# reglab/aquaculture

Hardware: AMD Instinct MI355X
Metric: 640px tiles/sec (whole node) YOLOv5m bf16 (higher is better)
Workload: dtype bf16

## Files before the change

### aquaculture_amd/csrc/bottleneck.hip

```cpp
#include "conv_device.h"

using namespace aqdev;

namespace {

struct BtlParams {
    const char* in;
    char* out;
    const char* w;
    const float* bias;
    int in_ld_b, out_ld_b;
    int B, H, W;
    int tiles_x, tiles_y, n_tiles;
    int shortcut;
    unsigned long long* debug;
    const char* zero;
};

template <int MBW, int MSPLIT, int NW, int TW, int KT, bool W1REG, bool RESG> struct BtlGeom {
    static constexpr int C = 16 * MBW * MSPLIT;
    static constexpr int CB = C / 8;
    static constexpr int PG = NW / MSPLIT;
    static constexpr int TH = 4 * PG;
    static constexpr int PH = TH + 2, PW = TW + 2, PP = PH * PW;
// ... 503 lines not shown

void btl_asm_pack(const float* w1, const float* w2, bf16_t* dst) {
    const int C = 48;
    static const int pairs[5][2] = {{0, 1}, {3, 4}, {6, 7}, {2, 5}, {8, -1}};
    for (int s = 0; s < 2; ++s)
        for (int m = 0; m < 3; ++m)
            for (int lane = 0; lane < 64; ++lane, dst += 8) {
                const int co = 16 * m + (lane & 15), blk = 4 * s + (lane >> 4);
                for (int e = 0; e < 8; ++e) dst[e] = blk < 6 ? aq_f2bf(w1[(size_t)co * C + blk * 8 + e]) : aq_f2bf(0.0f);
            }
    for (int s = 0; s < 14; ++s)
        for (int m = 0; m < 3; ++m)
            for (int lane = 0; lane < 64; ++lane, dst += 8) {
                const int co = 16 * m + (lane & 15), g = lane >> 4;
                int tap, c0;
                if (s < 9) { tap = s; c0 = 8 * g; }
                else { tap = pairs[s - 9][g >> 1]; c0 = 32 + 8 * (g & 1); }
                for (int e = 0; e < 8; ++e) dst[e] = tap >= 0 ? aq_f2bf(w2[((size_t)co * 9 + tap) * C + c0 + e]) : aq_f2bf(0.0f);
            }
}

const unsigned char kBtl96AsmCode[] = {
#include "bottleneck96_asm_hsaco.inc"
};
constexpr size_t kBtl96AsmWBytes = (size_t)2 * (9 + 81) * 1024;

bool btl96_asm_fits(int C, int B, int H, int W, int in_ld, int out_ld) {
    static const bool off = [] { const char* e = getenv("AQ_BTL96_ASM"); return e && *e == '0'; }();
    if (C != 96 || off || !btl_asm_enabled() || btl_wide()) return false;
    const long long tx = (W + 15) / 16, ty = (H + 7) / 8, tpi = tx * ty, nt = tpi * B;
    if (tx < 2 || tpi < 2 || nt >= (1LL << 24) || nt * tpi >= (1LL << 32)) return false;
    if ((long long)B * H * W * in_ld * 2 >= (1LL << 30) || (long long)B * H * W * out_ld * 2 >= (1LL << 31)) return false;
    return true;
}

int launch_btl96_asm(const BtlParams& p, hipStream_t stream) {
    int cus = 0;
    AQ_CHECK_HIP(aq_cus(&cus));
    BtlAsmArgs a{};
    a.in = p.in; a.out = p.out; a.bias = p.bias;
    a.w = p.w;
    a.in_ld_b = p.in_ld_b; a.out_ld_b = p.out_ld_b; a.B = p.B; a.H = p.H; a.W = p.W;
    a.tiles_x = (p.W + 15) / 16;
    a.tpi = a.tiles_x * ((p.H + 7) / 8);
    a.ntiles = a.tpi * p.B;
    a.shortcut = p.shortcut;
    long long grid = cus;
    if (grid > a.ntiles) grid = a.ntiles;
    a.G = (int)grid;
    a.magic_tpi = (unsigned)((1ULL << 32) / (unsigned)a.tpi + 1);
    a.magic_tx = (unsigned)((1ULL << 32) / (unsigned)a.tiles_x + 1);
    a.in_bytes = (unsigned)(((long long)p.B * p.H * p.W - 1) * p.in_ld_b + 192);
    a.pad = (unsigned)(((long long)p.B * p.H * p.W - 1) * p.out_ld_b + 192);
    a.debug = aq_stamp_target((size_t)grid * 4 * 64);
    const char* exp_kernel = getenv("AQ_BTL96_ASM_KERNEL");
    char name[96];
    snprintf(name, sizeof name, "%s%s", exp_kernel && *exp_kernel ? exp_kernel : "bottleneck_asm_c96", a.debug ? "_stamped" : "");
    hipFunction_t fn = nullptr;
    AQ_CHECK_HIP(aq_asm_fn(kBtl96AsmCode, name, &fn, false));
    AQ_CHECK_HIP(aq_asm_launch(fn, (unsigned)grid, 256, &a, sizeof a, stream));
    return AQ_OK;
}

void btl96_asm_pack(const float* w1, const float* w2, bf16_t* dst) {
    const int C = 96;
    for (int h = 0; h < 2; ++h) {
        auto chan = [&](int m, int r) { return 48 * h + (m < 2 ? 8 * (r >> 2) + 4 * m + (r & 3) : 32 + 4 * (r >> 2) + (r & 3)); };
        for (int s = 0; s < 3; ++s)
            for (int m = 0; m < 3; ++m)
                for (int lane = 0; lane < 64; ++lane, dst += 8) {
                    const int co = chan(m, lane & 15), c0 = 32 * s + 8 * (lane >> 4);
                    for (int e = 0; e < 8; ++e) dst[e] = aq_f2bf(w1[(size_t)co * C + c0 + e]);
                }
        for (int tap = 0; tap < 9; ++tap)
            for (int s = 0; s < 3; ++s)
                for (int m = 0; m < 3; ++m)
                    for (int lane = 0; lane < 64; ++lane, dst += 8) {
                        const int co = chan(m, lane & 15), c0 = 32 * s + 8 * (lane >> 4);
                        for (int e = 0; e < 8; ++e) dst[e] = aq_f2bf(w2[((size_t)co * 9 + tap) * C + c0 + e]);
                    }
    }
}

}

extern "C" int aq_pack_bottleneck_weights(const float* w1_host, const float* w2_host, int C, void* packed_dev, size_t* bytes, void* stream) {
    BtlShape sh;
    AQ_REQUIRE(w1_host && w2_host && bytes && btl_shape(C, &sh), "pack_bottleneck: C must be 16, 32, 48, 64 or 96 (got %d)", C);
    const int cb = C / 8, ks1 = (cb + 3) / 4, ks2 = (9 * cb + 3) / 4;
    const size_t frags = (size_t)sh.msplit * (ks1 + ks2) * sh.mbw;
    const size_t hip_bytes = frags * 64 * 16;
    *bytes = hip_bytes + (C == 48 ? kBtlAsmWBytes : C == 96 ? kBtl96AsmWBytes : 0);
    if (!packed_dev) return AQ_OK;
    bf16_t* host = (bf16_t*)calloc(1, *bytes);
    AQ_REQUIRE(host, "pack_bottleneck: out of host memory");
    for (int mh = 0; mh < sh.msplit; ++mh)
        for (int s = 0; s < ks1 + ks2; ++s)
            for (int m = 0; m < sh.mbw; ++m)
                for (int lane = 0; lane < 64; ++lane) {
                    const int co = (mh * sh.mbw + m) * 16 + (lane & 15), g = lane >> 4;
                    bf16_t* dst = host + ((((size_t)mh * (ks1 + ks2) + s) * sh.mbw + m) * 64 + lane) * 8;
                    if (s < ks1) {
                        const int blk = 4 * s + g;
                        if (blk < cb)
                            for (int e = 0; e < 8; ++e) dst[e] = aq_f2bf(w1_host[(size_t)co * C + blk * 8 + e]);
                    } else {
                        const int blk = 4 * (s - ks1) + g;
                        if (blk < 9 * cb) {
                            const int tap = blk / cb, c8 = blk % cb;
                            for (int e = 0; e < 8; ++e) dst[e] = aq_f2bf(w2_host[((size_t)co * 9 + tap) * C + c8 * 8 + e]);
                        }
                    }
                }
    if (C == 48) btl_asm_pack(w1_host, w2_host, (bf16_t*)((char*)host + hip_bytes));
    if (C == 96) btl96_asm_pack(w1_host, w2_host, (bf16_t*)((char*)host + hip_bytes));
    hipError_t e = hipMemcpyAsync(packed_dev, host, *bytes, hipMemcpyHostToDevice, (hipStream_t)stream);
    if (e == hipSuccess) e = hipStreamSynchronize((hipStream_t)stream);
    free(host);
    AQ_CHECK_HIP(e);
    return AQ_OK;
}

extern "C" int aq_bottleneck(const void* in_dev, int in_ld, int in_choff, void* out_dev, int out_ld, int out_choff, int C,
                             const void* packed_w_dev, const float* bias_dev, int B, int H, int W, int shortcut, void* stream) {
    BtlShape sh;
    AQ_REQUIRE(in_dev && out_dev && packed_w_dev && bias_dev, "bottleneck: null pointer");
    AQ_REQUIRE(btl_shape(C, &sh), "bottleneck: C must be 16, 32, 48, 64 or 96 (got %d)", C);
    AQ_REQUIRE(B > 0 && H > 0 && W > 0, "bottleneck: empty input");
    AQ_REQUIRE(in_ld % 8 == 0 && out_ld % 8 == 0 && in_choff % 8 == 0 && out_choff % 8 == 0 && in_choff + C <= in_ld && out_choff + C <= out_ld,
               "bottleneck: channel slices must be 8-aligned and inside their rows");
    AQ_REQUIRE((long long)B * H * W < (1LL << 31), "bottleneck: batch too large");
    BtlParams p{};
    p.in = (const char*)in_dev + (size_t)in_choff * 2; p.in_ld_b = in_ld * 2;
    p.out = (char*)out_dev + (size_t)out_choff * 2; p.out_ld_b = out_ld * 2;
    {
        const char* i0 = (const char*)in_dev; const char* i1 = i0 + (size_t)B * H * W * in_ld * 2;
        const char* o0 = (const char*)out_dev; const char* o1 = o0 + (size_t)B * H * W * out_ld * 2;
        AQ_REQUIRE(o1 <= i0 || i1 <= o0, "bottleneck: output overlaps input");
    }
    p.w = (const char*)packed_w_dev; p.bias = bias_dev;
    p.B = B; p.H = H; p.W = W; p.shortcut = shortcut;
    p.zero = aq_zero_page();
    AQ_REQUIRE(p.zero, "bottleneck: zero page allocation failed");
    const hipStream_t st = (hipStream_t)stream;
    if (btl_asm_fits(C, B, H, W, in_ld, out_ld)) {
        BtlShape sh48;
        btl_shape(48, &sh48);
        p.w += (size_t)sh48.msplit * ((48 / 8 + 3) / 4 + (9 * 48 / 8 + 3) / 4) * sh48.mbw * 64 * 16;
        return launch_btl_asm(p, st);
    }
    if (btl96_asm_fits(C, B, H, W, in_ld, out_ld)) {
        const int cb = 96 / 8, ks1 = (cb + 3) / 4, ks2 = (9 * cb + 3) / 4;
        p.w += (size_t)sh.msplit * (ks1 + ks2) * sh.mbw * 64 * 16;
        return launch_btl96_asm(p, st);
    }
    switch (C) {
        case 16: return launch_btl<1, 1, 4, 32, 0, false, false>(p, st);
        case 32: return launch_btl<2, 1, 4, 16, 0, false, false>(p, st);
        case 48: return btl_wide() ? launch_btl<3, 1, 4, 16, 0, false, false>(p, st) : launch_btl<1, 3, 12, 16, 0, true, false>(p, st);
        case 64: return launch_btl<4, 1, 4, 16, 3, false, false>(p, st);
        default: return btl_wide() ? launch_btl<3, 2, 4, 16, 3, false, false>(p, st) : launch_btl<1, 6, 12, 16, 12, true, true>(p, st);
    }
}
```

### aquaculture_amd/csrc/engine.cpp

```cpp
#include "aq_common.h"
#include <unistd.h>
#include <string>

#include <cstdarg>
#include <cstdio>
#include <cstdlib>
#include <cstring>
#include <string>
#include <atomic>
#include <dlfcn.h>
#include <vector>

namespace {
thread_local char g_err[512] = "";
}

void aq_set_error(const char* fmt, ...) {
    va_list ap;
    va_start(ap, fmt);
    vsnprintf(g_err, sizeof(g_err), fmt, ap);
    va_end(ap);
}

extern "C" const char* aq_last_error(void) { return g_err; }
extern "C" int aq_version(void) { return 8; }

namespace {

inline size_t align_up(size_t v, size_t a) { return (v + a - 1) / a * a; }
constexpr size_t kAlign = 256;
constexpr int kCoutSlack = 256;

struct Roctx {
    int (*push)(const char*) = nullptr;
    int (*pop)() = nullptr;
    bool tried = false;
    bool on() {
        if (!tried) {
            tried = true;
            const char* v = getenv("AQ_ROCTX");
            if (v && *v == '1') {
                void* h = dlopen("librocprofiler-sdk-roctx.so", RTLD_NOW | RTLD_GLOBAL);
                if (!h) h = dlopen("libroctx64.so", RTLD_NOW | RTLD_GLOBAL);
                if (h) {
                    push = (int (*)(const char*))dlsym(h, "roctxRangePushA");
                    pop = (int (*)())dlsym(h, "roctxRangePop");
                }
            }
        }
        return push && pop;
    }
} g_roctx;

constexpr int kCountStride = 1024;

struct PackedW {
    void* w = nullptr;
    float* bias = nullptr;
    int kgroups = 0, kgroups_pad = 0, G = 0, cout_rows = 0;
    bool x3 = false;
    void* w_direct = nullptr;
    int direct_cfg = -1;
    void* w_head = nullptr;
    void* w_pl8 = nullptr;
    float* sb_pl8 = nullptr;
    void* w_f8 = nullptr;
    float* sb_f8 = nullptr;
    float act_scale = 0.0f;
    int f8_consumer = -1;
    std::vector<float> w_host, b_host;
};

void pack_host(const float* w, int cout, int k, int cin, int precision, std::vector<unsigned char>& out,
               int* kgroups, int* kgroups_pad, int* G, int* cout_rows) {
    const int eb = aq_elem_bytes(precision);
    const int g = cin * eb / 16;
    const int kg = k * k * g;
    const int kgp = (kg + 7) / 8 * 8;
    const int rows = (cout + kCoutSlack + 31) / 32 * 32;
    out.assign((size_t)rows * kgp * 16, 0);
    const int kelems = k * k * cin;
    for (int co = 0; co < cout; ++co) {
        unsigned char* dst = out.data() + (size_t)co * kgp * 16;
        const float* src = w + (size_t)co * kelems;
        if (precision == AQ_FP32) {
            memcpy(dst, src, (size_t)kelems * 4);
        } else {
            bf16_t* d = (bf16_t*)dst;
            for (int e = 0; e < kelems; ++e) d[e] = aq_f2bf(src[e]);
        }
    }
    *kgroups = kg; *kgroups_pad = kgp; *G = g; *cout_rows = rows;
}

uint16_t f2h(float f) {
    _Float16 h = (_Float16)f;
    uint16_t u;
    memcpy(&u, &h, 2);
    return u;
}
float h2f(uint16_t u) {
    _Float16 h;
    memcpy(&h, &u, 2);
    return (float)h;
}

void pack_host_x3(const float* w, const float* bias, int cout, int k, int cin, std::vector<unsigned char>& out, std::vector<float>& bias_scale,
                  int* kgroups, int* kgroups_pad, int* G, int* cout_rows) {
    const int g = cin * 4 / 16;
    const int kg = k * k * g;
    const int kgp = (kg + 7) / 8 * 8;
    const int rows = (cout + kCoutSlack + 31) / 32 * 32;
    out.assign((size_t)rows * kgp * 16, 0);
    bias_scale.assign((size_t)2 * rows, 0.0f);
    for (int r = 0; r < rows; ++r) bias_scale[rows + r] = 1.0f;
    const int kelems = k * k * cin;
    for (int co = 0; co < cout; ++co) {
        const float* src = w + (size_t)co * kelems;
        float amax = 0.0f;
        for (int e = 0; e < kelems; ++e) amax = fmaxf(amax, fabsf(src[e]));
        int sexp = 0;
        if (amax > 0.0f && std::isfinite(amax)) {
            int ex = 0;
            frexpf(amax, &ex);
            sexp = 15 - ex;
            sexp = sexp > 60 ? 60 : (sexp < -60 ? -60 : sexp);
        }
        const float sc = ldexpf(1.0f, sexp);
        bias_scale[co] = bias ? bias[co] * sc : 0.0f;
        bias_scale[rows + co] = ldexpf(1.0f, -sexp);
        uint16_t* dst = (uint16_t*)(out.data() + (size_t)co * kgp * 16);
        for (int e0 = 0; e0 < kelems; e0 += 8) {
            for (int e = 0; e < 8; ++e) {
                const float v = src[e0 + e] * sc;
                const uint16_t hi = f2h(v);
                dst[2 * e0 + e] = hi;
                dst[2 * e0 + 8 + e] = f2h(v - h2f(hi));
            }
        }
    }
    *kgroups = kg; *kgroups_pad = kgp; *G = g; *cout_rows = rows;
}

struct TensorPlace { size_t offset = 0; size_t bytes = 0; int h = 0, w = 0, elem = 0; };

}

struct aq_engine {
    int device = 0;
    aq_model_desc desc{};
    std::vector<aq_tensor_desc> tensors;
    std::vector<aq_op_desc> ops;
    std::vector<PackedW> packed;
// ... 155 lines not shown
    const int out_f32 = e->tensors[op.dst.tensor].dtype == AQ_T_F32;
    ConvParams p{};
    p.in = tptr(e, ws, tiles, op.src.tensor) + (size_t)op.src.ch_off * eb;
    p.in_ld_b = e->tensors[op.src.tensor].channels * eb;
    p.out = tptr(e, ws, tiles, op.dst.tensor) + (size_t)op.dst.ch_off * pd.elem;
    p.out_ld_b = e->tensors[op.dst.tensor].channels * pd.elem;
    if (op.res.tensor >= 0) {
        p.res = tptr(e, ws, tiles, op.res.tensor) + (size_t)op.res.ch_off * eb;
        p.res_ld_b = e->tensors[op.res.tensor].channels * eb;
    }
    p.w = (const char*)pw.w; p.bias = pw.bias; p.zero = (const char*)e->zero_page;
    p.B = B; p.H = ps.h; p.W = ps.w; p.Ho = pd.h; p.Wo = pd.w;
    p.cout = op.dst.channels;
    p.k = op.k; p.stride = op.stride; p.pad = op.pad; p.taps = op.k * op.k;
    p.G = pw.G; p.kgroups = pw.kgroups; p.kgroups_pad = pw.kgroups_pad; p.nchunks = pw.kgroups_pad / 8;
    p.npix = B * pd.h * pd.w;
    p.act = op.act;
    int cfg = force_cfg >= 0 ? force_cfg : e->conv_cfg[oi];
    if (cfg < 0 && tt) cfg = tt->cfg[oi];
    if (cfg == AQ_CONV_CFG_DIRECT3X3S2) {
        if (pw.direct_cfg != cfg) { aq_set_error("conv op %d has no direct 3x3/s2 form", oi); return AQ_ERR_INVALID; }
        note_launch(e, oi, AQ_FAM_DIRECT3X3S2, cfg);
        return aq_conv3x3s2_direct(tptr(e, ws, tiles, op.src.tensor), e->tensors[op.src.tensor].channels, op.src.ch_off,
                                   tptr(e, ws, tiles, op.dst.tensor), e->tensors[op.dst.tensor].channels, op.dst.ch_off,
                                   op.src.channels, op.dst.channels, pw.w_direct, pw.bias, B, ps.h, ps.w, op.act, stream);
    }
    if (cfg == AQ_CONV_CFG_PL3X3) {
        if (pw.direct_cfg != cfg) { aq_set_error("conv op %d has no planar 3x3 form", oi); return AQ_ERR_INVALID; }
        const int ld = e->tensors[op.src.tensor].channels;
        note_launch(e, oi, pw.w_pl8 && aq_conv3x3_pl_w8_supported(op.src.channels, op.dst.channels, B, ps.h, ps.w) ? AQ_FAM_PL3X3_W8 : AQ_FAM_PL3X3, cfg);
        if (pw.w_pl8 && aq_conv3x3_pl_w8_supported(op.src.channels, op.dst.channels, B, ps.h, ps.w))
            return aq_conv3x3_pl_w8(tptr(e, ws, tiles, op.src.tensor) + (size_t)op.src.ch_off * 2, (long long)ld * 2, 16, op.src.channels,
                                    tptr(e, ws, tiles, op.dst.tensor), e->tensors[op.dst.tensor].channels, op.dst.ch_off, op.dst.channels,
                                    op.res.tensor >= 0 ? tptr(e, ws, tiles, op.res.tensor) : nullptr,
                                    op.res.tensor >= 0 ? e->tensors[op.res.tensor].channels : 0, op.res.ch_off,
                                    pw.w_pl8, pw.sb_pl8, B, ps.h, ps.w, op.act, stream);
        return aq_conv3x3_pl_at(tptr(e, ws, tiles, op.src.tensor) + (size_t)op.src.ch_off * 2, (long long)ld * 2, 16, op.src.channels,
                                tptr(e, ws, tiles, op.dst.tensor), e->tensors[op.dst.tensor].channels, op.dst.ch_off, op.dst.channels,
                                op.res.tensor >= 0 ? tptr(e, ws, tiles, op.res.tensor) : nullptr,
                                op.res.tensor >= 0 ? e->tensors[op.res.tensor].channels : 0, op.res.ch_off,
                                pw.w_direct, pw.bias, B, ps.h, ps.w, op.act, tt ? tt->B : B, stream);
    }
    if (cfg == AQ_CONV_CFG_PL3X3S2) {
        if (pw.direct_cfg != cfg) { aq_set_error("conv op %d has no planar 3x3/s2 form", oi); return AQ_ERR_INVALID; }
        if (!aq_conv3x3_pl_s2_supported(op.src.channels, op.dst.channels, B, ps.h, ps.w)) {
            aq_set_error("conv op %d: planar 3x3/s2 does not fit %d x %d x %d", oi, B, ps.h, ps.w);
            return AQ_ERR_INVALID;
        }
        note_launch(e, oi, AQ_FAM_PL3X3S2, cfg);
        return aq_conv3x3_pl_s2(tptr(e, ws, tiles, op.src.tensor), e->tensors[op.src.tensor].channels, op.src.ch_off, op.src.channels,
                                tptr(e, ws, tiles, op.dst.tensor), e->tensors[op.dst.tensor].channels, op.dst.ch_off, op.dst.channels,
                                pw.w_direct, pw.bias, B, ps.h, ps.w, op.act, stream);
    }
    if (cfg == AQ_CONV_CFG_DIRECT1X1) {
        if (pw.direct_cfg != cfg) { aq_set_error("conv op %d has no direct 1x1 form", oi); return AQ_ERR_INVALID; }
        note_launch(e, oi, AQ_FAM_DIRECT1X1, cfg);
        return aq_conv1x1_direct(tptr(e, ws, tiles, op.src.tensor), e->tensors[op.src.tensor].channels, op.src.ch_off,
                                 tptr(e, ws, tiles, op.dst.tensor), e->tensors[op.dst.tensor].channels, op.dst.ch_off,
                                 op.src.channels, op.dst.channels, pw.w_direct, pw.bias, (long long)B * pd.h * pd.w, op.act, stream);
    }
    if (cfg == AQ_CONV_CFG_ASM1X1) {
        if (pw.direct_cfg != cfg) { aq_set_error("conv op %d has no assembly 1x1 form", oi); return AQ_ERR_INVALID; }
        note_launch(e, oi, AQ_FAM_ASM1X1, cfg);
        return aq_conv1x1_asm(tptr(e, ws, tiles, op.src.tensor), e->tensors[op.src.tensor].channels, op.src.ch_off,
                              tptr(e, ws, tiles, op.dst.tensor), e->tensors[op.dst.tensor].channels, op.dst.ch_off,
                              op.src.channels, op.dst.channels, pw.w_direct, pw.bias, (long long)B * pd.h * pd.w, op.act, stream);
    }
    if (cfg < 0) cfg = aq_conv_pick_config(p.cout, p.npix, prec);
    if (pw.x3) p.x3_off = pw.cout_rows;
    note_launch(e, oi, AQ_FAM_IGEMM_OR_HALO, cfg);
    return aq_launch_conv(p, pw.x3 ? (int)AQ_F16X3 : prec, out_f32, cfg, stream);
}

bool heads_fused(const aq_engine* e) {
    int n_heads = 0;
    for (size_t oi = 0; oi < e->ops.size(); ++oi)
        if (e->ops[oi].kind == AQ_OP_CONV && e->ops[oi].level >= 0) {
            ++n_heads;
            if (!e->packed[oi].w_head) return false;
        }
    return n_heads == 3;
}

struct AugRun {
    int pass;
    const aq_augment_pass* ps;
    int H0, W0;
    const aq_tap* ytab;
    const aq_tap* xtab;
};

int run_plan(aq_engine* e, const uint8_t* tiles, int B, int H, int W, void* ws, size_t ws_bytes,
             float* pred_out, aq_det* dets, int32_t* counts, float conf, float iou, int max_det, hipStream_t stream,
             int first = 0, int last = -1, const AugRun* ar = nullptr) {
    AQ_REQUIRE(e && tiles && ws, "infer: null pointer");
    const int n_ops = (int)e->ops.size();
    if (last < 0) last = n_ops;
    AQ_REQUIRE(0 <= first && first <= last && last <= n_ops, "run_ops: range [%d, %d) is not inside the plan's %d ops", first, last, n_ops);
    int rc = AQ_OK;
    if (!ar) {
        rc = layout(e, B, H, W);
        if (rc) return rc;
        if (ws_bytes < e->total_bytes) {
            aq_set_error("workspace too small: need %zu bytes, got %zu", e->total_bytes, ws_bytes);
            return AQ_ERR_WORKSPACE;
        }
    }
    const bool scaled = ar && ar->pass > 0;
    const int aug_base = ar ? ar->ps->out_first - ar->ps->keep_first : 0;
    const float aug_scale = ar ? ar->ps->scale : 1.0f, aug_flip_w = ar && ar->ps->flip ? (float)ar->W0 : 0.0f;
    e->last_ws = ws; e->last_tiles = tiles;
    const int prec = e->desc.precision;
    const bool whole = first == 0 && last == n_ops;
    hipEvent_t* ev = nullptr;
    if (whole && !ar && e->prof && e->ring > 0) ev = e->ev.data() + (size_t)(e->prof_calls % e->ring) * (n_ops + 1);
    float* pred = pred_out ? pred_out : (float*)((char*)ws + e->off_pred);
    int32_t* cand = (int32_t*)((char*)ws + e->off_cand);
    int32_t* cand_count = (int32_t*)((char*)ws + e->off_cand_count);
    float* cand_rows = (float*)((char*)ws + e->off_cand_rows);
    const char* use_sd = getenv("AQ_STEMDOWN");
    const bool stemdown = use_sd && *use_sd == '1' && prec == AQ_BF16 && n_ops > 2 && e->ops[0].kind == AQ_OP_STEM && e->ops[1].kind == AQ_OP_DOWNBLOCK &&
                          e->ops[0].dst.channels == 48 && e->ops[1].src.tensor == e->ops[0].dst.tensor && e->ops[1].src.ch_off == e->ops[0].dst.ch_off &&
                          aq_stemdown_supported(H, W) && ((uintptr_t)tiles & 3) == 0 && !scaled;
    const bool fuse_heads = dets != nullptr && heads_fused(e);
    bool heads_started = ar != nullptr;
    int heads_done = 0;
    for (int oi = 0; oi < first; ++oi)
        if (fuse_heads && e->ops[oi].kind == AQ_OP_CONV && e->ops[oi].level >= 0) {
            heads_started = true;
            ++heads_done;
        }
    for (int oi = first; oi < last; ++oi) {
        const aq_op_desc& op = e->ops[oi];
        if (ev) AQ_CHECK_HIP(hipEventRecord(ev[oi], stream));
        const bool mark = g_roctx.on();
        if (mark) {
            char name[96];
            snprintf(name, sizeof name, "aq op %02d kind %d: %d -> %d ch, k%d s%d%s", oi, op.kind, op.src.channels, op.dst.channels, op.k, op.stride,
                     op.level >= 0 ? " (detect head)" : "");
            g_roctx.push(name);
        }
        switch (op.kind) {
        case AQ_OP_PREPROCESS:
            if (scaled)
                rc = aq_preprocess_s2d_scaled(tiles, ar->H0, ar->W0, ar->ytab, ar->xtab, ar->ps->h, ar->ps->w, tptr(e, ws, tiles, op.dst.tensor), B, H, W,
                                              prec, stream);
            else
                rc = aq_preprocess_s2d(tiles, tptr(e, ws, tiles, op.dst.tensor), B, H, W, prec, stream);
            break;
        case AQ_OP_CONV:
            if (ar && op.level >= 0 && !((ar->ps->level_mask >> op.level) & 1)) {
                note_launch(e, oi, AQ_FAM_NONE);
                break;
            }
            if (fuse_heads && op.level >= 0) {
                int32_t* wide = (int32_t*)((char*)ws + e->off_cand_wide);
                if (!heads_started) {
                    AQ_CHECK_HIP(hipMemsetAsync(wide, 0, sizeof(int32_t) * B * kCountStride, stream));
                    heads_started = true;
                }
                const TensorPlace& pl = e->place[op.src.tensor];
                int off = 0;
                for (int l = 0; l < op.level; ++l) off += e->desc.na * (H / (int)e->desc.stride[l]) * (W / (int)e->desc.stride[l]);
                float anchors[8 * 2];
                for (int a = 0; a < e->desc.na; ++a) {
                    anchors[2 * a] = e->desc.anchors_px[op.level][a][0];
                    anchors[2 * a + 1] = e->desc.anchors_px[op.level][a][1];
                }
                note_launch(e, oi, AQ_FAM_HEAD_DECODE);
                if (ar) {
                    rc = aq_head_decode_aug(tptr(e, ws, tiles, op.src.tensor), e->tensors[op.src.tensor].channels, op.src.ch_off, op.src.channels,
                                            e->packed[oi].w_head, B, pl.h, pl.w, aug_base + off, e->desc.stride[op.level], anchors, e->desc.nc, e->desc.na,
                                            conf, aug_scale, aug_flip_w, cand, cand_rows, wide, kCountStride, e->N, stream);
                    break;
                }
                rc = aq_head_decode(tptr(e, ws, tiles, op.src.tensor), e->tensors[op.src.tensor].channels, op.src.ch_off, op.src.channels,
                                    e->packed[oi].w_head, B, pl.h, pl.w, off, e->desc.stride[op.level], anchors, e->desc.nc, e->desc.na, conf,
                                    cand, cand_rows, wide, kCountStride, e->N, stream);
                if (!rc && ++heads_done == 3) rc = aq_head_counts_gather(wide, kCountStride, cand_count, B, stream);
                break;
            }
            rc = run_conv(e, oi, ws, tiles, B, stream);
            if (!rc && e->calib_amax && e->tensors[op.dst.tensor].dtype == AQ_T_ACT && prec == AQ_BF16 && op.dst.channels % 8 == 0) {
                const TensorPlace& pdc = e->place[op.dst.tensor];
                rc = aq_absmax_bf16(tptr(e, ws, tiles, op.dst.tensor), e->tensors[op.dst.tensor].channels, op.dst.ch_off, op.dst.channels,
                                    (long long)B * pdc.h * pdc.w, e->calib_amax + oi, stream);
            }
            break;
        case AQ_OP_STEM:
            note_launch(e, oi, AQ_FAM_STEM);
            if (stemdown) break;
            if (scaled) {
                rc = aq_stem_conv_scaled(tiles, ar->H0, ar->W0, ar->ytab, ar->xtab, ar->ps->h, ar->ps->w, tptr(e, ws, tiles, op.dst.tensor),
                                         e->tensors[op.dst.tensor].channels, op.dst.ch_off, op.dst.channels, e->packed[oi].w, e->packed[oi].bias,
                                         B, H, W, op.act, prec, stream);
                break;
            }
            rc = aq_stem_conv(tiles, tptr(e, ws, tiles, op.dst.tensor), e->tensors[op.dst.tensor].channels, op.dst.ch_off,
                              op.dst.channels, e->packed[oi].w, e->packed[oi].bias, B, H, W, op.act, prec, stream);
            break;
        case AQ_OP_BOTTLENECK: {
            note_launch(e, oi, AQ_FAM_BOTTLENECK);
            const TensorPlace& pl = e->place[op.src.tensor];
            rc = aq_bottleneck(tptr(e, ws, tiles, op.src.tensor), e->tensors[op.src.tensor].channels, op.src.ch_off,
                               tptr(e, ws, tiles, op.dst.tensor), e->tensors[op.dst.tensor].channels, op.dst.ch_off,
                               op.src.channels, e->packed[oi].w, e->packed[oi].bias, B, pl.h, pl.w, op.res.tensor >= 0, stream);
            break;
        }
        case AQ_OP_DOWNBLOCK: {
            note_launch(e, oi, AQ_FAM_DOWNBLOCK);
            const TensorPlace& pl = e->place[op.src.tensor];
            if (stemdown && oi == 1) {
                rc = aq_stemdown(tiles, tptr(e, ws, tiles, op.dst.tensor), e->tensors[op.dst.tensor].channels, op.dst.ch_off,
                                 e->packed[0].w, e->packed[0].bias, e->packed[oi].w, e->packed[oi].bias, B, H, W, stream);
                break;
            }
            rc = aq_downblock(tptr(e, ws, tiles, op.src.tensor), e->tensors[op.src.tensor].channels, op.src.ch_off,
                              tptr(e, ws, tiles, op.dst.tensor), e->tensors[op.dst.tensor].channels, op.dst.ch_off,
                              e->packed[oi].w, e->packed[oi].bias, B, pl.h, pl.w, stream);
            break;
        }
        case AQ_OP_SPPF_POOL: {
            const TensorPlace& pl = e->place[op.src.tensor];
            rc = aq_sppf_pool(tptr(e, ws, tiles, op.src.tensor), e->tensors[op.src.tensor].channels, op.src.ch_off,
                              op.src.channels, B, pl.h, pl.w, prec, stream);
            break;
        }
        case AQ_OP_UPSAMPLE2X: {
            const TensorPlace& pl = e->place[op.src.tensor];
            rc = aq_upsample2x(tptr(e, ws, tiles, op.src.tensor), e->tensors[op.src.tensor].channels, op.src.ch_off,
                               tptr(e, ws, tiles, op.dst.tensor), e->tensors[op.dst.tensor].channels, op.dst.ch_off,
                               op.src.channels, B, pl.h, pl.w, prec, stream);
            break;
        }
        case AQ_OP_DECODE: {
            if (fuse_heads) break;
            const float* heads[3];
            for (int l = 0; l < 3; ++l) heads[l] = (const float*)tptr(e, ws, tiles, e->desc.head_tensor[l]);
            float anchors[3 * 8 * 2];
            for (int l = 0; l < 3; ++l)
                for (int a = 0; a < e->desc.na; ++a) {
                    anchors[(l * e->desc.na + a) * 2] = e->desc.anchors_px[l][a][0];
                    anchors[(l * e->desc.na + a) * 2 + 1] = e->desc.anchors_px[l][a][1];
                }
            const bool want_nms = dets != nullptr;
            if (ar) {
                rc = aq_detect_decode_aug(heads, e->tensors[e->desc.head_tensor[0]].channels, B, H, W, e->desc.nc, e->desc.na, anchors,
                                          e->desc.stride, ar->ps->level_mask, aug_base, e->N, aug_scale, aug_flip_w, want_nms ? nullptr : pred,
                                          conf, want_nms ? cand : nullptr, want_nms ? cand_rows : nullptr, want_nms ? cand_count : nullptr,
                                          e->N, stream);
                break;
            }
            rc = aq_detect_decode(heads, e->tensors[e->desc.head_tensor[0]].channels, B, H, W, e->desc.nc, e->desc.na,
                                  anchors, e->desc.stride, want_nms ? nullptr : pred, conf, want_nms ? cand : nullptr,
                                  want_nms ? cand_rows : nullptr, want_nms ? cand_count : nullptr, e->N, stream);
            break;
        }
        case AQ_OP_NMS:
            if (dets && !ar)
                rc = aq_nms_opts(cand_rows, e->N, B, e->N, e->desc.nc, conf, iou, max_det, cand, cand_count, e->N,
                                 (char*)ws + e->off_nms, dets, counts, e->nms_agnostic, e->nms_cls_lo, e->nms_cls_hi, stream);
            break;
        default:
            aq_set_error("unknown op kind %d", op.kind);
            rc = AQ_ERR_INVALID;
        }
        if (mark) g_roctx.pop();
        if (rc) return rc;
    }
    if (ev) {
        AQ_CHECK_HIP(hipEventRecord(ev[n_ops], stream));
        e->prof_calls++;
    }
    return AQ_OK;
}

int run_augment(aq_engine* e, const uint8_t* tiles, int B, int H, int W, void* ws, size_t ws_bytes, float* pred_out, aq_det* dets,
                int32_t* counts, float conf, float iou, int max_det, hipStream_t stream) {
    AQ_REQUIRE(e && tiles && ws, "augment: null pointer");
    for (const PackedW& pw : e->packed)
        AQ_REQUIRE(!pw.w_f8, "augment: this engine has fp8 activation scales installed; they were calibrated at one geometry, and the "
                             "augmented passes run at three");
    int rc = layout(e, B, H, W, true);
    if (rc) return rc;
    AQ_REQUIRE(e->aug[0].hp == H && e->aug[0].wp == W, "augment: internal error, the passes do not belong to the %d x %d layout", H, W);
    if (ws_bytes < e->total_bytes) {
// ... 60 lines not shown
                                       float* bias_scale_dev, size_t* bias_floats, void* stream) {
    AQ_REQUIRE(w && bytes && bias_floats, "pack_conv_weights_x3: null pointer");
    AQ_REQUIRE(cout > 0 && k > 0 && cin > 0 && cin % 8 == 0, "pack_conv_weights_x3: cin %d is not a multiple of 8", cin);
    std::vector<unsigned char> host;
    std::vector<float> bs;
    int kg, kgp, g, rows;
    pack_host_x3(w, bias, cout, k, cin, host, bs, &kg, &kgp, &g, &rows);
    *bytes = host.size();
    *bias_floats = bs.size();
    if (!packed_dev) return AQ_OK;
    AQ_REQUIRE(bias && bias_scale_dev, "pack_conv_weights_x3: null pointer");
    AQ_CHECK_HIP(hipMemcpyAsync(packed_dev, host.data(), host.size(), hipMemcpyHostToDevice, (hipStream_t)stream));
    AQ_CHECK_HIP(hipMemcpyAsync(bias_scale_dev, bs.data(), bs.size() * sizeof(float), hipMemcpyHostToDevice, (hipStream_t)stream));
    AQ_CHECK_HIP(hipStreamSynchronize((hipStream_t)stream));
    return AQ_OK;
}

extern "C" int aq_conv2d(const void* in_dev, int in_ld, int in_choff, int cin, void* out_dev, int out_ld, int out_choff,
                         int cout, const void* res_dev, int res_ld, int res_choff, const void* packed_w_dev,
                         const float* bias_dev, int B, int H, int W, int k, int stride, int pad, int act, int precision,
                         int out_f32, const void* zero_page_dev, void* stream) {
    AQ_REQUIRE(in_dev && out_dev && packed_w_dev && bias_dev && zero_page_dev, "conv2d: null pointer");
    const int eb = aq_elem_bytes(precision);
    const int oeb = (eb == 4 || out_f32) ? 4 : 2;
    AQ_REQUIRE((cin * eb) % 16 == 0 && (in_ld * eb) % 16 == 0 && (in_choff * eb) % 16 == 0,
               "conv2d: input channels must be whole 16-byte groups (cin=%d ld=%d off=%d)", cin, in_ld, in_choff);
    AQ_REQUIRE(cout % 8 == 0 && out_choff % 8 == 0 && out_ld % 8 == 0, "conv2d: cout/out_choff/out_ld must be multiples of 8");
    AQ_REQUIRE(!res_dev || (res_choff % 8 == 0 && res_ld % 8 == 0), "conv2d: residual slice must be 8-channel aligned");
    AQ_REQUIRE(k >= 1 && k * k <= 25 && stride >= 1 && pad >= 0, "conv2d: unsupported k=%d stride=%d pad=%d", k, stride, pad);
    AQ_REQUIRE(precision == AQ_BF16 || precision == AQ_FP32 || precision == AQ_F16X3, "conv2d: bad precision %d", precision);
    AQ_REQUIRE(precision != AQ_F16X3 || cin % 8 == 0, "conv2d: split mode needs cin %% 8 == 0");
    ConvParams p{};
    p.x3_off = precision == AQ_F16X3 ? (cout + kCoutSlack + 31) / 32 * 32 : 0;
    p.in = (const char*)in_dev + (size_t)in_choff * eb; p.in_ld_b = in_ld * eb;
    p.out = (char*)out_dev + (size_t)out_choff * oeb; p.out_ld_b = out_ld * oeb;
    if (res_dev) { p.res = (const char*)res_dev + (size_t)res_choff * eb; p.res_ld_b = res_ld * eb; }
    p.w = (const char*)packed_w_dev; p.bias = bias_dev; p.zero = (const char*)zero_page_dev;
    p.B = B; p.H = H; p.W = W;
    p.Ho = (H + 2 * pad - k) / stride + 1; p.Wo = (W + 2 * pad - k) / stride + 1;
    AQ_REQUIRE(p.Ho > 0 && p.Wo > 0, "conv2d: empty output");
    p.cout = cout; p.k = k; p.stride = stride; p.pad = pad; p.taps = k * k;
    p.G = cin * eb / 16; p.kgroups = p.taps * p.G; p.kgroups_pad = (p.kgroups + 7) / 8 * 8; p.nchunks = p.kgroups_pad / 8;
    p.npix = B * p.Ho * p.Wo; p.act = act;
    int cfg = aq_conv_pick_config(cout, p.npix, precision);
    const char* forced = getenv("AQ_CONV_CFG");
    if (forced && *forced) cfg = atoi(forced);
    return aq_launch_conv(p, precision, out_f32, cfg, (hipStream_t)stream);
}

extern "C" int aq_engine_create(const aq_model_desc* d, int device, aq_engine** out) {
    AQ_REQUIRE(d && out, "engine_create: null pointer");
    AQ_REQUIRE(d->n_ops > 0 && d->n_tensors > 0 && d->ops && d->tensors, "engine_create: empty plan");
    AQ_REQUIRE(d->nl == 3 && d->na >= 1 && d->na <= 8 && d->nc >= 1, "engine_create: unsupported head nl=%d na=%d nc=%d", d->nl, d->na, d->nc);
    AQ_REQUIRE(d->precision == AQ_BF16 || d->precision == AQ_FP32 || d->precision == AQ_BF16_W8 || d->precision == AQ_F16X3,
               "engine_create: bad precision %d", d->precision);
    {
        static std::atomic<int> first_device{-1};
        int expected = -1;
        if (!first_device.compare_exchange_strong(expected, device))
            AQ_REQUIRE(expected == device, "engine_create: this process already runs engines on device %d; device %d needs its own process", expected, device);
    }
    AQ_CHECK_HIP(hipSetDevice(device));
    aq_engine* e = new aq_engine();
    e->device = device;
    aq_model_desc compute_desc = *d;
    const bool w8 = d->precision == AQ_BF16_W8;
    if (w8) compute_desc.precision = AQ_BF16;
    const bool x3 = d->precision == AQ_F16X3;
    if (x3) compute_desc.precision = AQ_FP32;
    d = &compute_desc;
    e->desc = *d;
    e->tensors.assign(d->tensors, d->tensors + d->n_tensors);
    e->ops.assign(d->ops, d->ops + d->n_ops);
    e->desc.tensors = e->tensors.data();
    e->desc.ops = e->ops.data();
    e->packed.resize(e->ops.size());
    e->conv_cfg.assign(e->ops.size(), -1);
    const int eb = aq_elem_bytes(d->precision);
    auto fail = [&](int rc) { aq_engine_destroy(e); return rc; };
    if (hipMalloc(&e->zero_page, 4096) != hipSuccess || hipMemset(e->zero_page, 0, 4096) != hipSuccess) {
        aq_set_error("engine_create: zero page allocation failed");
        return fail(AQ_ERR_NOMEM);
    }
    for (size_t oi = 0; oi < e->ops.size(); ++oi) {
        aq_op_desc& op = e->ops[oi];
        for (const aq_slice* s : {&op.src, &op.dst}) {
            if (op.kind == AQ_OP_DECODE || op.kind == AQ_OP_NMS) continue;
            if (s->tensor < 0 || s->tensor >= d->n_tensors || s->ch_off < 0 ||
                s->ch_off + s->channels > e->tensors[s->tensor].channels) {
                aq_set_error("engine_create: op %zu has a slice outside its tensor", oi);
                return fail(AQ_ERR_INVALID);
            }
        }
        if (op.kind == AQ_OP_STEM) {
            PackedW& pw = e->packed[oi];
            size_t nb = 0;
            std::vector<float> bias(64, 0.0f);
            if (!op.weight || !op.bias || op.k != 6 || op.stride != 2 || op.pad != 2 || op.src.channels != 3 || op.dst.channels > 64 ||
                aq_pack_stem_weights(op.weight, op.dst.channels, d->precision, nullptr, &nb, nullptr) != AQ_OK) {
                aq_set_error("engine_create: stem op %zu unsupported (needs k=6 s=2 p=2, 3 -> <=64 channels)", oi);
                return fail(AQ_ERR_INVALID);
            }
            memcpy(bias.data(), op.bias, sizeof(float) * op.dst.channels);
            if (hipMalloc(&pw.w, nb) != hipSuccess || hipMalloc((void**)&pw.bias, bias.size() * sizeof(float)) != hipSuccess) {
                aq_set_error("engine_create: stem weight allocation failed");
                return fail(AQ_ERR_NOMEM);
            }
            if (aq_pack_stem_weights(op.weight, op.dst.channels, d->precision, pw.w, &nb, nullptr) != AQ_OK ||
                hipMemcpy(pw.bias, bias.data(), bias.size() * sizeof(float), hipMemcpyHostToDevice) != hipSuccess) {
                aq_set_error("engine_create: stem weight upload failed");
                return fail(AQ_ERR_HIP);
            }
            op.weight = nullptr; op.bias = nullptr;
            continue;
        }
        if (op.kind == AQ_OP_BOTTLENECK) {
            PackedW& pw = e->packed[oi];
            const int C = op.src.channels;
            size_t nb = 0;
            if (!op.weight || !op.bias || d->precision != AQ_BF16 || op.k != 3 || op.stride != 1 || op.pad != 1 || op.dst.channels != C ||
                op.src.tensor == op.dst.tensor ||
                aq_pack_bottleneck_weights(op.weight, op.weight + (size_t)C * C, C, nullptr, &nb, nullptr) != AQ_OK) {
                aq_set_error("engine_create: bottleneck op %zu unsupported (bf16, C in {16,32,48,64,96}, distinct src/dst tensors)", oi);
                return fail(AQ_ERR_INVALID);
            }
            if (hipMalloc(&pw.w, nb) != hipSuccess || hipMalloc((void**)&pw.bias, 2 * C * sizeof(float)) != hipSuccess) {
                aq_set_error("engine_create: bottleneck weight allocation failed");
                return fail(AQ_ERR_NOMEM);
            }
            if (aq_pack_bottleneck_weights(op.weight, op.weight + (size_t)C * C, C, pw.w, &nb, nullptr) != AQ_OK ||
                hipMemcpy(pw.bias, op.bias, 2 * C * sizeof(float), hipMemcpyHostToDevice) != hipSuccess) {
                aq_set_error("engine_create: bottleneck weight upload failed");
                return fail(AQ_ERR_HIP);
            }
            op.weight = nullptr; op.bias = nullptr;
            continue;
        }
        if (op.kind == AQ_OP_DOWNBLOCK) {
            PackedW& pw = e->packed[oi];
            size_t nb = 0;
            if (!op.weight || !op.bias || d->precision != AQ_BF16 || op.k != 3 || op.stride != 2 || op.pad != 1 || op.src.channels != 48 ||
                op.dst.channels != 96 || aq_pack_downblock_weights(op.weight, op.weight + (size_t)96 * 9 * 48, nullptr, &nb, nullptr) != AQ_OK) {
                aq_set_error("engine_create: downblock op %zu unsupported (bf16, 3x3/s2 48 -> 96 then 1x1 96 -> 96)", oi);
                return fail(AQ_ERR_INVALID);
            }
            if (hipMalloc(&pw.w, nb) != hipSuccess || hipMalloc((void**)&pw.bias, 192 * sizeof(float)) != hipSuccess) {
                aq_set_error("engine_create: downblock weight allocation failed");
                return fail(AQ_ERR_NOMEM);
            }
            if (aq_pack_downblock_weights(op.weight, op.weight + (size_t)96 * 9 * 48, pw.w, &nb, nullptr) != AQ_OK ||
                hipMemcpy(pw.bias, op.bias, 192 * sizeof(float), hipMemcpyHostToDevice) != hipSuccess) {
                aq_set_error("engine_create: downblock weight upload failed");
                return fail(AQ_ERR_HIP);
            }
            op.weight = nullptr; op.bias = nullptr;
            continue;
        }
        if (op.kind != AQ_OP_CONV) continue;
        if (!op.weight || !op.bias || (op.src.channels * eb) % 16 != 0 || op.dst.channels % 8 != 0 || op.dst.ch_off % 8 != 0 || op.k * op.k > 25) {
            aq_set_error("engine_create: conv op %zu unsupported (cin=%d cout=%d k=%d)", oi, op.src.channels, op.dst.channels, op.k);
            return fail(AQ_ERR_INVALID);
        }
        std::vector<unsigned char> host;
        PackedW& pw = e->packed[oi];
        std::vector<float> bias;
        if (x3 && op.src.channels % 8 == 0) {
// ... 34 lines not shown
                aq_set_error("engine_create: assembly 1x1 weight upload failed (op %zu)", oi);
                return fail(AQ_ERR_HIP);
            }
            pw.direct_cfg = AQ_CONV_CFG_ASM1X1;
        }
        if (d->precision == AQ_BF16 && op.k == 3 && op.stride == 2 && op.pad == 1 && op.res.tensor < 0 && e->tensors[op.dst.tensor].dtype == AQ_T_ACT &&
            aq_conv3x3s2_direct_supported(op.src.channels, op.dst.channels)) {
            size_t nb = 0;
            if (aq_pack_conv3x3s2_direct(op.weight, op.src.channels, op.dst.channels, nullptr, &nb, nullptr) != AQ_OK ||
                hipMalloc(&pw.w_direct, nb) != hipSuccess ||
                aq_pack_conv3x3s2_direct(op.weight, op.src.channels, op.dst.channels, pw.w_direct, &nb, nullptr) != AQ_OK) {
                aq_set_error("engine_create: direct 3x3/s2 weight upload failed (op %zu)", oi);
                return fail(AQ_ERR_HIP);
            }
            pw.direct_cfg = AQ_CONV_CFG_DIRECT3X3S2;
        }
        const char* no_pl2 = getenv("AQ_DISABLE_PL3X3S2");
        if (d->precision == AQ_BF16 && op.k == 3 && op.stride == 2 && op.pad == 1 && op.res.tensor < 0 && e->tensors[op.dst.tensor].dtype == AQ_T_ACT &&
            pw.direct_cfg < 0 && op.src.ch_off % 8 == 0 && e->tensors[op.src.tensor].channels % 8 == 0 && !(no_pl2 && *no_pl2 == '1') &&
            aq_conv3x3_pl_s2_supported(op.src.channels, op.dst.channels, 1, 2, 2)) {
            size_t nb = 0;
            if (aq_pack_conv3x3_pl_s2(op.weight, op.src.channels, op.dst.channels, nullptr, &nb, nullptr) != AQ_OK ||
                hipMalloc(&pw.w_direct, nb) != hipSuccess ||
                aq_pack_conv3x3_pl_s2(op.weight, op.src.channels, op.dst.channels, pw.w_direct, &nb, nullptr) != AQ_OK) {
                aq_set_error("engine_create: planar 3x3/s2 weight upload failed (op %zu)", oi);
                return fail(AQ_ERR_HIP);
            }
            pw.direct_cfg = AQ_CONV_CFG_PL3X3S2;
        }
        const char* no_pl = getenv("AQ_DISABLE_PL3X3");
        if (d->precision == AQ_BF16 && op.k == 3 && op.stride == 1 && op.pad == 1 && e->tensors[op.dst.tensor].dtype == AQ_T_ACT &&
            op.src.ch_off % 8 == 0 && aq_conv3x3_pl_supported(op.src.channels, op.dst.channels) && !(no_pl && *no_pl == '1')) {
            size_t nb = 0;
            if (aq_pack_conv3x3_pl(op.weight, op.src.channels, op.dst.channels, nullptr, &nb, nullptr) != AQ_OK ||
                hipMalloc(&pw.w_direct, nb) != hipSuccess ||
                aq_pack_conv3x3_pl(op.weight, op.src.channels, op.dst.channels, pw.w_direct, &nb, nullptr) != AQ_OK) {
                aq_set_error("engine_create: planar 3x3 weight upload failed (op %zu)", oi);
                return fail(AQ_ERR_HIP);
            }
            pw.direct_cfg = AQ_CONV_CFG_PL3X3;
            const char* use_w8 = getenv("AQ_PL_W8");
            if (w8 && use_w8 && *use_w8 == '1') {
                if (aq_pack_conv3x3_pl_w8(op.weight, op.bias, op.src.channels, op.dst.channels, nullptr, &nb, nullptr, nullptr) == AQ_OK &&
                    hipMalloc(&pw.w_pl8, nb) == hipSuccess && hipMalloc((void**)&pw.sb_pl8, 2048 * sizeof(float)) == hipSuccess) {
                    if (aq_pack_conv3x3_pl_w8(op.weight, op.bias, op.src.channels, op.dst.channels, pw.w_pl8, &nb, pw.sb_pl8, nullptr) != AQ_OK) {
                        (void)hipFree(pw.w_pl8); (void)hipFree(pw.sb_pl8);
                        pw.w_pl8 = nullptr; pw.sb_pl8 = nullptr;
                    }
                }
            }
        }
        const char* no_hf = getenv("AQ_DISABLE_HEAD_FUSION");
        if (d->precision == AQ_BF16 && op.level >= 0 && op.k == 1 && op.stride == 1 && !op.act && op.res.tensor < 0 &&
            op.dst.channels >= d->na * (d->nc + 5) && op.dst.channels <= 32 && aq_head_decode_supported(op.src.channels, d->na, d->nc) && !(no_hf && *no_hf == '1')) {
            size_t nb = 0;
            if (aq_pack_head_weights(op.weight, op.bias, op.src.channels, op.dst.channels, nullptr, &nb, nullptr) != AQ_OK ||
                hipMalloc(&pw.w_head, nb) != hipSuccess ||
                aq_pack_head_weights(op.weight, op.bias, op.src.channels, op.dst.channels, pw.w_head, &nb, nullptr) != AQ_OK) {
                aq_set_error("engine_create: fused head weight upload failed (op %zu)", oi);
                return fail(AQ_ERR_HIP);
            }
        }
        if (d->precision == AQ_BF16 && op.kind == AQ_OP_CONV && op.k == 3 && op.stride == 1 && op.pad == 1 && e->packed[oi].direct_cfg == AQ_CONV_CFG_PL3X3 &&
            aq_conv3x3_pl_f8_supported(op.src.channels, op.dst.channels, 1, 8, 8)) {
            e->packed[oi].w_host.assign(op.weight, op.weight + (size_t)op.dst.channels * 9 * op.src.channels);
            e->packed[oi].b_host.assign(op.bias, op.bias + op.dst.channels);
        }
        op.weight = nullptr; op.bias = nullptr;
    }
    *out = e;
    return AQ_OK;
}

extern "C" void aq_engine_destroy(aq_engine* e) {
    if (!e) return;
    for (PackedW& pw : e->packed) {
        if (pw.w) (void)hipFree(pw.w);
        if (pw.w_direct) (void)hipFree(pw.w_direct);
        if (pw.w_head) (void)hipFree(pw.w_head);
        if (pw.w_pl8) (void)hipFree(pw.w_pl8);
        if (pw.w_f8) (void)hipFree(pw.w_f8);
        if (pw.sb_f8) (void)hipFree(pw.sb_f8);
        if (pw.sb_pl8) (void)hipFree(pw.sb_pl8);
        if (pw.bias) (void)hipFree(pw.bias);
    }
    if (e->zero_page) (void)hipFree(e->zero_page);
    for (hipEvent_t ev : e->ev) (void)hipEventDestroy(ev);
    delete e;
}

extern "C" int aq_engine_workspace_bytes(aq_engine* e, int max_batch, int H, int W, size_t* bytes) {
    AQ_REQUIRE(e && bytes, "workspace_bytes: null pointer");
    int rc = layout(e, max_batch, H, W);
    if (rc) return rc;
    *bytes = e->total_bytes;
    return AQ_OK;
}

extern "C" int aq_engine_infer(aq_engine* e, const uint8_t* tiles_dev, int B, int H, int W, void* ws, size_t ws_bytes,
                               aq_det* dets_dev, int32_t* counts_dev, float conf, float iou, int max_det, void* stream) {
    AQ_REQUIRE(dets_dev && counts_dev, "infer: null output pointer");
    AQ_REQUIRE(max_det > 0 && conf >= 0.f && conf <= 1.f && iou >= 0.f && iou <= 1.f,
               "infer: bad thresholds conf=%g iou=%g max_det=%d", conf, iou, max_det);
    return run_plan(e, tiles_dev, B, H, W, ws, ws_bytes, nullptr, dets_dev, counts_dev, conf, iou, max_det, (hipStream_t)stream);
}

extern "C" int aq_engine_workspace_bytes_augment(aq_engine* e, int max_batch, int H, int W, size_t* bytes) {
    AQ_REQUIRE(e && bytes, "workspace_bytes_augment: null pointer");
    int rc = layout(e, max_batch, H, W, true);
    if (rc) return rc;
    *bytes = e->total_bytes;
    return AQ_OK;
}

extern "C" int aq_engine_infer_augment(aq_engine* e, const uint8_t* tiles_dev, int B, int H, int W, void* ws, size_t ws_bytes,
                                       aq_det* dets_dev, int32_t* counts_dev, float conf, float iou, int max_det, void* stream) {
    AQ_REQUIRE(dets_dev && counts_dev, "infer_augment: null output pointer");
    AQ_REQUIRE(max_det > 0 && conf >= 0.f && conf <= 1.f && iou >= 0.f && iou <= 1.f,
               "infer_augment: bad thresholds conf=%g iou=%g max_det=%d", conf, iou, max_det);
    return run_augment(e, tiles_dev, B, H, W, ws, ws_bytes, nullptr, dets_dev, counts_dev, conf, iou, max_det, (hipStream_t)stream);
}

extern "C" int aq_engine_forward_raw_augment(aq_engine* e, const uint8_t* tiles_dev, int B, int H, int W, void* ws, size_t ws_bytes,
                                             float* pred_dev, void* stream) {
    AQ_REQUIRE(pred_dev, "forward_raw_augment: null output pointer");
    return run_augment(e, tiles_dev, B, H, W, ws, ws_bytes, pred_dev, nullptr, nullptr, 0.f, 0.f, 1, (hipStream_t)stream);
}

extern "C" int aq_engine_last_launch_augment(aq_engine* e, int pass, int op, int* family, int* cfg) {
    AQ_REQUIRE(e && family && pass >= 0 && pass < 3 && op >= 0 && op < (int)e->ops.size(), "last_launch_augment: bad argument");
    const bool have = e->aug_family[pass].size() == e->ops.size();
    *family = have ? e->aug_family[pass][op] : AQ_FAM_NONE;
    if (cfg) *cfg = have ? e->aug_cfg[pass][op] : -1;
    return AQ_OK;
}

extern "C" int aq_engine_run_ops(aq_engine* e, const uint8_t* tiles_dev, int B, int H, int W, void* ws, size_t ws_bytes, int first, int last,
                                 float conf, float iou, int max_det, aq_det* dets_dev, int32_t* counts_dev, void* stream) {
    AQ_REQUIRE(dets_dev && counts_dev, "run_ops: null output pointer");
    AQ_REQUIRE(max_det > 0 && conf >= 0.f && conf <= 1.f && iou >= 0.f && iou <= 1.f,
               "run_ops: bad thresholds conf=%g iou=%g max_det=%d", conf, iou, max_det);
    AQ_REQUIRE(e && first >= 0 && first <= last && last <= (int)e->ops.size(), "run_ops: range [%d, %d) is not inside the plan", first, last);
    return run_plan(e, tiles_dev, B, H, W, ws, ws_bytes, nullptr, dets_dev, counts_dev, conf, iou, max_det, (hipStream_t)stream, first, last);
}

extern "C" int aq_engine_forward_raw(aq_engine* e, const uint8_t* tiles_dev, int B, int H, int W, void* ws, size_t ws_bytes,
                                     float* pred_dev, void* stream) {
    AQ_REQUIRE(pred_dev, "forward_raw: null output pointer");
    return run_plan(e, tiles_dev, B, H, W, ws, ws_bytes, pred_dev, nullptr, nullptr, 0.f, 0.f, 1, (hipStream_t)stream);
}

extern "C" int aq_engine_calibrate_amax(aq_engine* e, const uint8_t* tiles_dev, int B, int H, int W, void* ws, size_t ws_bytes,
                                        float* amax_host, int n_ops, void* stream_) {
    hipStream_t stream = (hipStream_t)stream_;
    AQ_REQUIRE(e && tiles_dev && ws && amax_host && n_ops == (int)e->ops.size(), "calibrate_amax: expected %d entries", e ? (int)e->ops.size() : 0);
    AQ_REQUIRE(e->desc.precision == AQ_BF16, "calibrate_amax: bf16 engines only");
    int rc = layout(e, B, H, W);
    if (rc) return rc;
    if (ws_bytes < e->total_bytes) { aq_set_error("calibrate_amax: workspace too small"); return AQ_ERR_WORKSPACE; }
    float* dev = nullptr;
    AQ_CHECK_HIP(hipMalloc((void**)&dev, sizeof(float) * n_ops));
    hipError_t he = hipMemsetAsync(dev, 0, sizeof(float) * n_ops, stream);
    e->calib_amax = dev;
    if (he == hipSuccess) rc = run_plan(e, tiles_dev, B, H, W, ws, ws_bytes, (float*)((char*)ws + e->off_pred), nullptr, nullptr, 0.f, 0.f, 1, stream);
    e->calib_amax = nullptr;
    if (he == hipSuccess && !rc) he = hipMemcpyAsync(amax_host, dev, sizeof(float) * n_ops, hipMemcpyDeviceToHost, stream);
// ... 251 lines not shown
```

### aquaculture_amd/csrc/gen_bottleneck_asm.py

```python
#!/usr/bin/env python3
import sys

C = 48
CB = 6
PXB = 96
PW = 18
PP = PW * PW
BUF = 32768
X0, T0 = 0, 2 * BUF
W1_OFF = 4 * BUF
BIAS_OFF = W1_OFF + 6 * 1024
LDS_BYTES = BIAS_OFF + 512
NBLK1 = 21
KS2 = 14

KSTEPS = [("A", t) for t in range(9)] + [("P1", 0, 1), ("P1", 3, 4), ("P1", 6, 7), ("P2", 2, 5), ("P1", 8, -1)]
assert len(KSTEPS) == KS2

ARG = dict(inp=0, out=8, w=16, bias=24, in_ld=32, out_ld=36, B=40, H=44, W=48, tiles_x=52, tpi=56, ntiles=60, shortcut=64, G=68,
           magic_tpi=72, magic_tx=76, in_bytes=80, pad=84, debug=88)
ARG_BYTES = 96


class Regs:
    def __init__(self, prefix, limit):
        self.prefix, self.limit, self.next, self.names = prefix, limit, 0, {}

    def alloc(self, name, n=1, align=1):
        self.next = (self.next + align - 1) // align * align
        base = self.next
        self.next += n
        assert self.next <= self.limit, f"out of {self.prefix} registers at {name}"
        self.names[name] = (base, n)
        return base


import os as _os
W16 = _os.environ.get("AQ_GEN_BTL_W16", "0") == "1"
V = Regs("v", 256)
S = Regs("s", 100)

S.alloc("karg", 2)
S.alloc("wg")
S.alloc("pad0")
for nm in ("inp", "out", "w", "bias"):
    S.alloc(nm, 2, 2)
for nm in ("in_ld", "out_ld", "B", "H", "W", "tiles_x", "tpi", "ntiles", "shortcut", "G", "magic_tpi", "magic_tx", "in_bytes", "pad"):
    S.alloc(nm)
S.alloc("debug", 2, 2)
S.alloc("srd", 4, 4)
for nm in ("wave", "group", "tmp0", "tmp1", "tmp2", "tmp3", "tmp4", "tmp5",
           "d_tile", "d_ok", "d_b", "d_y0", "d_x0",
           "b_ok", "b_b", "b_y0", "b_x0",
           "c_ok", "c_b", "c_y0", "c_x0",
           "dma_lds", "org", "y0m1", "x0m1", "interior", "wlim", "rowok0", "rowok1", "blk2"):
    S.alloc(nm)
S.alloc("klog2e2", 2, 2)
S.alloc("kone2", 2, 2)
S.alloc("orow0", 2, 2)
S.alloc("orow1", 2, 2)
S.alloc("irow0", 2, 2)
S.alloc("irow1", 2, 2)
S.alloc("colmask", 2, 2)
S.alloc("mask0", 2, 2)
S.alloc("mask1", 2, 2)
S.alloc("sa", 2, 2)
S.alloc("t64", 2, 2)
S.alloc("st_last", 2, 2)
S.alloc("st_acc", 12, 2)

V.alloc("tid")
V.alloc("l15")
V.alloc("W2", 4 * 3 * KS2, 4)
for nm in ("cA", "cP1", "cP2", "xb", "tw", "bb", "w1a", "pre0", "pre1", "pre2", "pre3", "vin", "vout"):
    V.alloc(nm)
V.alloc("ACC", 24, 4)
V.alloc("F", 16, 4)
V.alloc("P", 28, 4)


def s(name, i=0):
    b, n = S.names[name]
    assert i < n
    return f"s{b + i}"


def s2(name, i=0):
    b, n = S.names[name]
    assert i + 1 < n and (b + i) % 2 == 0
    return f"s[{b + i}:{b + i + 1}]"


def s4(name):
    b, n = S.names[name]
    assert n == 4 and b % 4 == 0
    return f"s[{b}:{b + 3}]"


def v(name, i=0):
    b, n = V.names[name]
    assert i < n, (name, i)
    return f"v{b + i}"


def vr(name, i, cnt):
    b, n = V.names[name]
    assert i + cnt <= n, (name, i, cnt)
    return f"v[{b + i}:{b + i + cnt - 1}]"


def w2(s_, m):
    return vr("W2", 4 * (3 * s_ + m), 4)


def acc(j, m):
    return vr("ACC", 4 * (3 * j + m), 4)


out = []
_uid = [0]
STAMPED = [False]
OPT = dict(stagger=True, nosilu=False, nomfma=False, nopk=False, nodma=False, nold=False, nost=False, prio=0, ntst=False, ntld=False)
PH_PROLOGUE, PH_DMA, PH_B, PH_C_MFMA, PH_C_EPI, PH_BARRIER = range(6)


def E(line="", comment=None):
    if OPT["nomfma"] and line.startswith("v_mfma"):
        return
    if (OPT["nodma"] and line.startswith("buffer_load_dwordx4")) or (OPT["nold"] and line.startswith("global_load_dwordx2")) or (OPT["nost"] and line.startswith("global_store_dwordx")):
        return
    if OPT["nosilu"] and line.split(" ")[0] in ("v_exp_f32", "v_rcp_f32", "v_pk_mul_f32", "v_pk_add_f32", "v_mul_f32", "v_add_f32"):
        return
    if OPT["nopk"] and line.split(" ")[0] in ("v_pk_mul_f32", "v_pk_add_f32"):
        op = "v_mul_f32" if "mul" in line else "v_add_f32"
        import re
        m_ = re.match(r"v_pk_\w+ v\[(\d+):\d+\], v\[(\d+):\d+\], (.*)$", line)
        d, a, rest = int(m_.group(1)), int(m_.group(2)), m_.group(3)
        for h in range(2):
            r2 = re.match(r"v\[(\d+):\d+\]$", rest)
            if r2:
                b_ = f"v{int(r2.group(1)) + h}"
            else:
                r3 = re.match(r"s\[(\d+):\d+\]$", rest)
                b_ = f"s{int(r3.group(1)) + h}"
            out.append(f"\t{op}_e64 v{d + h}, v{a + h}, {b_}")
        return
    if (OPT["ntst"] and line.startswith("global_store_dwordx")) or (OPT["ntld"] and line.startswith("global_load_dwordx2")):
        line += " nt"
    out.append(("\t" + line if line and not line.endswith(":") else line) + (f"\t; {comment}" if comment else ""))


def label(name):
    out.append(f"{name}:")


def uid(prefix):
    _uid[0] += 1
    return f".L{prefix}_{_uid[0]}"


def stamp(k):
    if not STAMPED[0]:
        return
    E(f"s_memtime {s2('t64')}")
    E("s_waitcnt lgkmcnt(0)")
    E(f"s_sub_u32 {s('tmp4')}, {s('t64')}, {s('st_last')}")
    E(f"s_subb_u32 {s('tmp5')}, {s('t64', 1)}, {s('st_last', 1)}")
    E(f"s_add_u32 {s('st_acc', 2 * k)}, {s('st_acc', 2 * k)}, {s('tmp4')}")
    E(f"s_addc_u32 {s('st_acc', 2 * k + 1)}, {s('st_acc', 2 * k + 1)}, {s('tmp5')}")
    E(f"s_mov_b64 {s2('st_last')}, {s2('t64')}")


def tap_off(t):
    return ((t // 3) * PW + t % 3) * PXB


def emit_decode(stage):
    skip = uid("dec")
    E(f"s_cmp_lt_u32 {s('d_tile')}, {s('ntiles')}")
    E(f"s_cselect_b32 {s('d_ok')}, 1, 0")
    E(f"s_cbranch_scc0 {skip}")
    E(f"s_mul_hi_u32 {s('d_b')}, {s('d_tile')}, {s('magic_tpi')}", "image = tile / tiles per image")
    E(f"s_mul_i32 {s('tmp0')}, {s('d_b')}, {s('tpi')}")
    E(f"s_sub_u32 {s('tmp0')}, {s('d_tile')}, {s('tmp0')}", "tile inside the image")
    E(f"s_mul_hi_u32 {s('tmp1')}, {s('tmp0')}, {s('magic_tx')}", "tile row")
    E(f"s_mul_i32 {s('tmp2')}, {s('tmp1')}, {s('tiles_x')}")
    E(f"s_sub_u32 {s('tmp2')}, {s('tmp0')}, {s('tmp2')}", "tile column")
    E(f"s_lshl_b32 {s('d_y0')}, {s('tmp1')}, 4")
    E(f"s_lshl_b32 {s('d_x0')}, {s('tmp2')}, 4")
    label(skip)


def emit_dma(temps_base=None):
    skip = uid("dma")
    E(f"s_cmp_eq_u32 {s('d_ok')}, 0")
    E(f"s_cbranch_scc1 {skip}")
    E(f"s_mul_i32 {s('tmp0')}, {s('d_b')}, {s('H')}")
    E(f"s_add_u32 {s('tmp0')}, {s('tmp0')}, {s('d_y0')}")
    E(f"s_sub_u32 {s('tmp0')}, {s('tmp0')}, 1")
    E(f"s_mul_i32 {s('tmp0')}, {s('tmp0')}, {s('W')}")
    E(f"s_add_u32 {s('tmp0')}, {s('tmp0')}, {s('d_x0')}")
    E(f"s_sub_u32 {s('tmp0')}, {s('tmp0')}, 1")
    E(f"s_mul_i32 {s('org')}, {s('tmp0')}, {s('in_ld')}")
    E(f"s_lshl_b32 {s('tmp1')}, {s('wave')}, 12")
    E(f"s_add_u32 {s('tmp1')}, {s('tmp1')}, {s('dma_lds')}")
# ... 41 lines not shown
    def mfmas(aset):
        for ks in range(2):
            for m in range(3):
                a = A0 + 12 * aset + 4 * m
                E(f"v_mfma_f32_16x16x32_bf16 v[{a}:{a + 3}], v[{P0 + 4 * (3 * ks + m)}:{P0 + 4 * (3 * ks + m) + 3}], v[{F0 + 4 * ks}:{F0 + 4 * ks + 3}], v[{a}:{a + 3}]")

    def silu_store(i, aset):
        regs = [A0 + 12 * aset + k for k in range(12)]
        if not interior:
            t0, t1, t2 = temps[8], temps[9], temps[10]
            E(f"s_lshl_b32 {s('tmp0')}, {s('wave')}, 4")
            E(f"s_add_u32 {s('tmp0')}, {s('tmp0')}, {128 * i}")
            E(f"v_add_u32 v{t0}, {s('tmp0')}, {v('l15')}", "patch pixel")
            E(f"v_mul_u32_u24 v{t1}, 3641, v{t0}")
            E(f"v_lshrrev_b32 v{t1}, 16, v{t1}", "patch row = pixel / 18")
            E(f"v_mul_u32_u24 v{t2}, 18, v{t1}")
            E(f"v_sub_u32 v{t2}, v{t0}, v{t2}", "patch column")
            E(f"v_add_u32 v{t1}, {s('y0m1')}, v{t1}", "image row (wraps below zero)")
            E(f"v_add_u32 v{t2}, {s('x0m1')}, v{t2}")
            E(f"v_cmp_gt_u32 {s2('sa')}, {s('H')}, v{t1}")
            E(f"v_cmp_gt_u32 vcc, {s('W')}, v{t2}")
            E(f"s_and_b64 vcc, vcc, {s2('sa')}")
        emit_silu(regs, temps)
        for k in range(0, 12, 2):
            E(f"v_pk_mul_f32 v[{regs[k]}:{regs[k] + 1}], v[{regs[k]}:{regs[k] + 1}], v[{temps[k]}:{temps[k] + 1}]")
        for k in range(6):
            E(f"v_cvt_pk_bf16_f32 v{temps[k]}, v{regs[2 * k]}, v{regs[2 * k] + 1}")
        if not interior:
            for k in range(6):
                E(f"v_cndmask_b32 v{temps[k]}, 0, v{temps[k]}, vcc")
        for m in range(3):
            E(f"ds_write_b64 {v('tw')}, v[{temps[2 * m]}:{temps[2 * m] + 1}] offset:{12288 * i + 32 * m}")

    reads(0, 0)
    E("s_waitcnt lgkmcnt(0)")
    mfmas(0)
    reads(1, 1)
    E("s_nop 7", "hz: MFMA result -> VALU read")
    silu_store(0, 0)
    E("s_waitcnt lgkmcnt(3)", "block 1's fragments and b1 (the three t writes behind them may still be on their way)")
    mfmas(1)
    no2 = uid("nob2")
    end = uid("pbe")
    E(f"s_cmp_eq_u32 {s('blk2')}, 0")
    E(f"s_cbranch_scc1 {no2}")
    reads(2, 0)
    E("s_nop 7", "hz: MFMA result -> VALU read")
    silu_store(1, 1)
    E("s_waitcnt lgkmcnt(3)")
    mfmas(0)
    E("s_nop 15", "hz: MFMA result -> VALU read")
    silu_store(2, 0)
    E(f"s_branch {end}")
    label(no2)
    E("s_nop 15", "hz: MFMA result -> VALU read")
    silu_store(1, 1)
    label(end)


def emit_phase_b_dispatch():
    skip = uid("pb")
    border = uid("pbb")
    E(f"s_cmp_eq_u32 {s('b_ok')}, 0")
    E(f"s_cbranch_scc1 {skip}")
    E(f"s_add_u32 {s('tmp0')}, {s('b_y0')}, 17")
    E(f"s_add_u32 {s('tmp1')}, {s('b_x0')}, 17")
    E(f"s_cmp_le_u32 {s('tmp0')}, {s('H')}")
    E(f"s_cselect_b32 {s('interior')}, 1, 0")
    E(f"s_cmp_le_u32 {s('tmp1')}, {s('W')}")
    E(f"s_cselect_b32 {s('tmp2')}, 1, 0")
    E(f"s_and_b32 {s('interior')}, {s('interior')}, {s('tmp2')}")
    E(f"s_min_u32 {s('tmp2')}, {s('b_y0')}, {s('b_x0')}")
    E(f"s_min_u32 {s('tmp2')}, {s('tmp2')}, 1", "1 when both origins are > 0")
    E(f"s_and_b32 {s('interior')}, {s('interior')}, {s('tmp2')}")
    E(f"s_cmp_eq_u32 {s('interior')}, 0")
    E(f"s_cbranch_scc1 {border}")
    emit_phase_b(True)
    E(f"s_branch {skip}")
    label(border)
    emit_phase_b(False)
    label(skip)


def emit_phase_c(dma_inside):
    skip = uid("pc")
    if dma_inside:
        have = uid("pch")
        E(f"s_cmp_eq_u32 {s('c_ok')}, 1")
        E(f"s_cbranch_scc1 {have}")
        emit_dma()
        E(f"s_branch {skip}")
        label(have)
    else:
        E(f"s_cmp_eq_u32 {s('c_ok')}, 0")
        E(f"s_cbranch_scc1 {skip}")
    P0 = V.names["P"][0]
    F0 = V.names["F"][0]
    A0 = V.names["ACC"][0]
    E(f"s_lshl_b32 {s('tmp0')}, {s('wave')}, 1")
    E(f"s_add_u32 {s('tmp0')}, {s('tmp0')}, {s('c_y0')}", "image row of the wave's first output row")
    E(f"s_cmp_lt_u32 {s('tmp0')}, {s('H')}")
    E(f"s_cselect_b32 {s('rowok0')}, 1, 0")
    E(f"s_add_u32 {s('tmp1')}, {s('tmp0')}, 1")
    E(f"s_cmp_lt_u32 {s('tmp1')}, {s('H')}")
    E(f"s_cselect_b32 {s('rowok1')}, 1, 0")
    E(f"s_mul_i32 {s('tmp1')}, {s('c_b')}, {s('H')}")
    E(f"s_add_u32 {s('tmp1')}, {s('tmp1')}, {s('tmp0')}")
    E(f"s_mul_i32 {s('tmp1')}, {s('tmp1')}, {s('W')}")
    E(f"s_add_u32 {s('tmp1')}, {s('tmp1')}, {s('c_x0')}", "pixel index of (row 0, x0)")
    for nm, ld, base in (("orow", "out_ld", "out"), ("irow", "in_ld", "inp")):
        E(f"s_mul_i32 {s('tmp2')}, {s('tmp1')}, {s(ld)}")
        E(f"s_mul_hi_u32 {s('tmp3')}, {s('tmp1')}, {s(ld)}")
        E(f"s_add_u32 {s(nm + '0')}, {s(base)}, {s('tmp2')}")
        E(f"s_addc_u32 {s(nm + '0', 1)}, {s(base, 1)}, {s('tmp3')}")
        E(f"s_mul_i32 {s('tmp2')}, {s('W')}, {s(ld)}")
        E(f"s_add_u32 {s(nm + '1')}, {s(nm + '0')}, {s('tmp2')}")
        E(f"s_addc_u32 {s(nm + '1', 1)}, {s(nm + '0', 1)}, 0")
    E(f"s_sub_u32 {s('wlim')}, {s('W')}, {s('c_x0')}", "columns of the tile inside the image")
    E(f"v_cmp_gt_u32 {s2('colmask')}, {s('wlim')}, {v('l15')}")
    E(f"s_cmp_eq_u32 {s('rowok0')}, 1")
    E(f"s_cselect_b64 {s2('mask0')}, {s2('colmask')}, 0")
    E(f"s_cmp_eq_u32 {s('rowok1')}, 1")
    E(f"s_cselect_b64 {s2('mask1')}, {s2('colmask')}, 0")
    nosc = uid("nosc")
    E(f"s_cmp_eq_u32 {s('shortcut')}, 0")
    E(f"s_cbranch_scc1 {nosc}")
    for j in range(2):
        E(f"s_mov_b64 exec, {s2('mask' + str(j))}")
        for m in range(3):
            E(f"global_load_dwordx2 v[{P0 + 2 * (3 * j + m)}:{P0 + 2 * (3 * j + m) + 1}], {v('vin')}, {s2('irow' + str(j))} offset:{32 * m}")
    E("s_mov_b64 exec, -1")
    label(nosc)
    if dma_inside:
        emit_dma(temps_base=P0 + 12)
    for j in range(2):
        for m in range(3):
            E(f"ds_read_b128 {acc(j, m)}, {v('bb')} offset:{192 + 64 * m}", "accumulators start from b2")

    ring = [F0 + 4 * i for i in range(4)] + [P0 + 12 + 4 * i for i in range(4)]
    PD = 3

    def frag_reads(k):
        kind = KSTEPS[k]
        for j in range(2):
            dst = ring[(2 * k + j) % 8]
            areg = "cA" if kind[0] == "A" else "c" + kind[0]
            E(f"ds_read_b128 v[{dst}:{dst + 3}], {v(areg)} offset:{tap_off(kind[1]) + j * PW * PXB}")

    for k in range(PD):
        frag_reads(k)
    if OPT["prio"]:
        E(f"s_setprio {OPT['prio']}")
    for k in range(KS2):
        if k + PD < KS2:
            frag_reads(k + PD)
        ahead = 2 * (min(KS2, k + PD + 1) - (k + 1))
        E(f"s_waitcnt lgkmcnt({ahead})")
        for m in range(3):
            for j in range(2):
                f = ring[(2 * k + j) % 8]
                E(f"v_mfma_f32_16x16x32_bf16 {acc(j, m)}, {w2(k, m)}, v[{f}:{f + 3}], {acc(j, m)}")
    if OPT["prio"]:
        E("s_setprio 0")
    stamp(PH_C_MFMA)
    E("s_nop 15", "hz: MFMA result -> VALU read")
    if dma_inside:
        w0, wd = uid("w0"), uid("wd")
        E(f"s_cmp_eq_u32 {s('d_ok')}, 0")
        E(f"s_cbranch_scc1 {w0}")
        E("s_waitcnt vmcnt(4)", "shortcut values (the four LDS-DMA instructions behind them stay in flight)")
        E(f"s_branch {wd}")
        label(w0)
        E("s_waitcnt vmcnt(0)")
        label(wd)
    else:
        E("s_waitcnt vmcnt(0)", "shortcut values (and, vmcnt being in order, this interval's LDS-DMA and the previous tile's stores)")
    stamp(PH_DMA)
    temps = [P0 + 12 + i for i in range(12)]
    plain, done = uid("pl"), uid("dn")
    if W16:
        E(f"s_mov_b32 {s('sa')}, 0xffff0000", "lanes with odd q")
        E(f"s_mov_b32 {s('sa', 1)}, 0xffff0000")
        E(f"s_mul_i32 {s('tmp4')}, {s('W')}, {s('out_ld')}")
        E(f"s_add_u32 {s('tmp4')}, {s('tmp4')}, {64 - 8 - 64}", "row 1's block 2 from row 0's address: + one image row - 8 (the store's own offset is 64)")
    E(f"s_cmp_eq_u32 {s('shortcut')}, 0")
    E(f"s_cbranch_scc1 {plain}")
    for with_sc in (True, False):
        if not with_sc:
            label(plain)
        for j in range(2):
            regs = [A0 + 12 * j + k for k in range(12)]
            emit_silu(regs, temps)
            for k in range(0, 12, 2):
                E(f"v_pk_mul_f32 v[{regs[k]}:{regs[k] + 1}], v[{regs[k]}:{regs[k] + 1}], v[{temps[k]}:{temps[k] + 1}]")
            if with_sc:
                for m in range(3):
                    sc = P0 + 2 * (3 * j + m)
                    E(f"v_lshlrev_b32 v{temps[4 * m]}, 16, v{sc}")
                    E(f"v_and_b32 v{temps[4 * m + 1]}, 0xffff0000, v{sc}")
                    E(f"v_lshlrev_b32 v{temps[4 * m + 2]}, 16, v{sc + 1}")
                    E(f"v_and_b32 v{temps[4 * m + 3]}, 0xffff0000, v{sc + 1}")
                for k in range(0, 12, 2):
                    E(f"v_pk_add_f32 v[{regs[k]}:{regs[k] + 1}], v[{regs[k]}:{regs[k] + 1}], v[{temps[k]}:{temps[k] + 1}]")
            if W16:
                for k in range(4):
                    E(f"v_cvt_pk_bf16_f32 v{temps[k]}, v{regs[2 * k]}, v{regs[2 * k] + 1}")
                for k in (4, 5):
                    E(f"v_cvt_pk_bf16_f32 v{A0 + 2 * j + k - 4}, v{regs[2 * k]}, v{regs[2 * k] + 1}")
                E(f"v_cndmask_b32 v{temps[6]}, 0, 24, {s2('sa')}")
                E(f"v_add_u32 v{temps[6]}, v{temps[6]}, {v('vout')}")
                E(f"v_permlane16_swap_b32 v{temps[0]}, v{temps[2]}")
                E(f"v_permlane16_swap_b32 v{temps[1]}, v{temps[3]}")
                E(f"s_mov_b64 exec, {s2('mask' + str(j))}")
                E(f"global_store_dwordx4 v{temps[6]}, v[{temps[0]}:{temps[3]}], {s2('orow' + str(j))}")
                E("s_mov_b64 exec, -1")
                if j == 0:
                    E("s_nop 0", "hz: store of more than 8 bytes -> VALU write of its data registers, 2 wait states on gfx940+ (row 1's SiLU starts in them)")
                if j == 1:
                    E(f"v_mov_b32 v{temps[7]}, {s('tmp4')}")
                    E(f"v_cndmask_b32 v{temps[7]}, 0, v{temps[7]}, {s2('sa')}")
                    E(f"v_add_u32 v{temps[7]}, v{temps[7]}, {v('vout')}")
                    E(f"v_permlane16_swap_b32 v{A0}, v{A0 + 2}")
                    E(f"v_permlane16_swap_b32 v{A0 + 1}, v{A0 + 3}")
                    E(f"s_andn2_b64 {s2('t64')}, {s2('mask0')}, {s2('sa')}")
                    E(f"s_and_b64 {s2('colmask')}, {s2('mask1')}, {s2('sa')}")
                    E(f"s_or_b64 exec, {s2('t64')}, {s2('colmask')}")
                    E(f"global_store_dwordx4 v{temps[7]}, v[{A0}:{A0 + 3}], {s2('orow0')} offset:64")
                    E("s_mov_b64 exec, -1")
                continue
            for k in range(6):
                E(f"v_cvt_pk_bf16_f32 v{temps[k]}, v{regs[2 * k]}, v{regs[2 * k] + 1}")
            E(f"s_mov_b64 exec, {s2('mask' + str(j))}")
            for m in range(3):
                E(f"global_store_dwordx2 {v('vout')}, v[{temps[2 * m]}:{temps[2 * m] + 1}], {s2('orow' + str(j))} offset:{32 * m}")
            E("s_mov_b64 exec, -1")
        if with_sc:
            E(f"s_branch {done}")
    label(done)
    stamp(PH_C_EPI)
    label(skip)


_kernel_no = [0]


def gen_kernel(name, stamped=False, **opt):
    global out
    out = []
    STAMPED[0] = stamped
    OPT.update(dict(stagger=True, nosilu=False, nomfma=False, nopk=False, nodma=False, nold=False, nost=False, prio=0, ntst=False, ntld=False))
    OPT.update(opt)
    _kernel_no[0] += 1
    _uid[0] = 100000 * _kernel_no[0]
    E(f"; fused Bottleneck, C = 48, 8 waves: generated by gen_bottleneck_asm.py -- do not edit")
    label(name)
    a0 = S.names["inp"][0]
    b0 = S.names["in_ld"][0]
    assert a0 % 4 == 0 and b0 == a0 + 8 and S.names["debug"][0] == b0 + 14
    E(f"s_load_dwordx8 s[{a0}:{a0 + 7}], {s2('karg')}, 0x0", "inp, out, w, bias")
    E(f"s_load_dwordx8 s[{b0}:{b0 + 7}], {s2('karg')}, 0x20", "in_ld .. ntiles")
    E(f"s_load_dwordx4 s[{b0 + 8}:{b0 + 11}], {s2('karg')}, 0x40", "shortcut, G, magic_tpi, magic_tx")
    E(f"s_load_dwordx4 s[{b0 + 12}:{b0 + 15}], {s2('karg')}, 0x50", "in_bytes, pad, debug")
    T = [V.names["P"][0] + i for i in range(28)]
    E(f"v_and_b32 v{T[0]}, 63, {v('tid')}", "lane")
    E(f"v_lshrrev_b32 v{T[1]}, 6, {v('tid')}")
    E("s_nop 1", "hz: VALU write -> v_readfirstlane")
    E(f"v_readfirstlane_b32 {s('wave')}, v{T[1]}")
    E(f"v_and_b32 {v('l15')}, 15, v{T[0]}")
    E(f"v_lshrrev_b32 v{T[2]}, 4, v{T[0]}", "g")
    if OPT["stagger"]:
        E(f"s_lshr_b32 {s('group')}, {s('wave')}, 2")
    else:
        E(f"s_mov_b32 {s('group')}, 0", "experiment: every wave runs phase C first (no stagger)")
    E(f"s_cmp_lt_u32 {s('wave')}, 5")
    E(f"s_cselect_b32 {s('blk2')}, 1, 0", "waves 0-4 own a third block of the patch (21 blocks)")
    E("s_waitcnt lgkmcnt(0)")
    E(f"s_mov_b32 {s('srd', 0)}, {s('inp')}")
    E(f"s_and_b32 {s('srd', 1)}, {s('inp', 1)}, 0xffff")
    E(f"s_mov_b32 {s('srd', 2)}, {s('in_bytes')}")
    E(f"s_mov_b32 {s('srd', 3)}, 0x00020000")
    E(f"s_mov_b32 {s('klog2e2')}, 0xbfb8aa3b", "-log2(e)")
    E(f"s_mov_b32 {s('klog2e2', 1)}, 0xbfb8aa3b")
    E(f"s_mov_b32 {s('kone2')}, 1.0")
    E(f"s_mov_b32 {s('kone2', 1)}, 1.0")
    if stamped:
        for k in range(12):
            E(f"s_mov_b32 {s('st_acc', k)}, 0")
        E(f"s_memtime {s2('st_last')}")
        E("s_waitcnt lgkmcnt(0)")
    E(f"s_mul_i32 {s('tmp0')}, {s('wave')}, {2 * PW * PXB}")
    E(f"s_add_u32 {s('tmp0')}, {s('tmp0')}, {T0 + BUF}")
    E(f"v_mul_u32_u24 v{T[3]}, {PXB}, {v('l15')}")
    E(f"v_add_u32 v{T[3]}, {s('tmp0')}, v{T[3]}", "pixel (2 wave, l15) of t patch 1")
    E(f"v_lshl_add_u32 {v('cA')}, v{T[2]}, 4, v{T[3]}", "+ 16 g: channel block g of the tap")
    E(f"v_and_b32 v{T[4]}, 1, v{T[2]}", "g & 1")
    E(f"v_lshrrev_b32 v{T[5]}, 1, v{T[2]}", "g >> 1: which tap of the pair")
    E(f"v_lshl_add_u32 v{T[6]}, v{T[4]}, 4, v{T[3]}")
    E(f"v_add_u32 v{T[6]}, 64, v{T[6]}", "channel block 4 + (g & 1)")
    E(f"v_mul_u32_u24 v{T[7]}, {PXB}, v{T[5]}")
    E(f"v_add_u32 {v('cP1')}, v{T[6]}, v{T[7]}", "second tap: one pixel to the right")
    E(f"v_mul_u32_u24 v{T[7]}, {PW * PXB}, v{T[5]}")
    E(f"v_add_u32 {v('cP2')}, v{T[6]}, v{T[7]}", "second tap: one patch row down")
    E(f"s_mul_i32 {s('tmp0')}, {s('wave')}, {16 * PXB}")
    E(f"v_mul_u32_u24 v{T[3]}, {PXB}, {v('l15')}")
    E(f"v_add_u32 v{T[3]}, {s('tmp0')}, v{T[3]}")
    E(f"v_lshl_add_u32 {v('xb')}, v{T[2]}, 4, v{T[3]}", "x patch 0 + 16 g")
    E(f"v_lshl_add_u32 {v('tw')}, v{T[2]}, 3, v{T[3]}")
    E(f"v_add_u32 {v('tw')}, {T0}, {v('tw')}", "t patch 0 + 8 g (four bf16 channels per lane and M block)")
    E(f"v_lshlrev_b32 {v('bb')}, 4, v{T[2]}")
    E(f"v_add_u32 {v('bb')}, {BIAS_OFF}, {v('bb')}")
    E(f"v_lshlrev_b32 {v('w1a')}, 4, v{T[0]}")
    E(f"v_add_u32 {v('w1a')}, {W1_OFF}, {v('w1a')}")
    for i in range(4):
        E(f"s_lshl_b32 {s('tmp0')}, {s('wave')}, 8")
        E(f"s_add_u32 {s('tmp0')}, {s('tmp0')}, {64 * i}")
        E(f"v_add_u32 v{T[3]}, {s('tmp0')}, v{T[0]}", "slot")
        E(f"v_mul_u32_u24 v{T[4]}, 10923, v{T[3]}")
        E(f"v_lshrrev_b32 v{T[4]}, 16, v{T[4]}", "pixel = slot / 6")
        E(f"v_mul_u32_u24 v{T[5]}, 6, v{T[4]}")
        E(f"v_sub_u32 v{T[5]}, v{T[3]}, v{T[5]}", "part")
        E(f"v_mul_u32_u24 v{T[6]}, 3641, v{T[4]}")
        E(f"v_lshrrev_b32 v{T[6]}, 16, v{T[6]}", "patch row")
        E(f"v_mul_u32_u24 v{T[7]}, {PW}, v{T[6]}")
        E(f"v_sub_u32 v{T[7]}, v{T[4]}, v{T[7]}", "patch column")
        E(f"v_mul_lo_u32 v{T[6]}, v{T[6]}, {s('W')}")
        E(f"v_add_u32 v{T[6]}, v{T[6]}, v{T[7]}")
        E(f"v_mul_lo_u32 v{T[6]}, v{T[6]}, {s('in_ld')}")
        E(f"v_lshl_add_u32 v{T[6]}, v{T[5]}, 4, v{T[6]}", "(row W + column) in_ld + 16 part")
        E(f"v_mov_b32 v{T[8]}, 0x80000000")
        E(f"v_cmp_gt_u32 vcc, {PP}, v{T[4]}")
        E(f"v_cndmask_b32 {v('pre' + str(i))}, v{T[8]}, v{T[6]}, vcc", "slots beyond the patch: outside the descriptor -> zeros")
    E(f"v_mul_lo_u32 v{T[3]}, {v('l15')}, {s('in_ld')}")
    E(f"v_lshl_add_u32 {v('vin')}, v{T[2]}, 3, v{T[3]}")
    E(f"v_mul_lo_u32 v{T[3]}, {v('l15')}, {s('out_ld')}")
    E(f"v_lshl_add_u32 {v('vout')}, v{T[2]}, 3, v{T[3]}")
    E(f"s_lshr_b32 {s('tmp0')}, {s('G')}, 3", "q")
    E(f"s_and_b32 {s('tmp1')}, {s('G')}, 7", "r")
    E(f"s_and_b32 {s('tmp2')}, {s('wg')}, 7", "xcd")
    E(f"s_add_u32 {s('tmp3')}, {s('tmp0')}, 1", "q + 1")
    E(f"s_cmp_lt_u32 {s('tmp2')}, {s('tmp1')}")
    E(f"s_cselect_b32 {s('d_tile')}, {s('tmp2')}, {s('tmp1')}", "min(xcd, r)")
    E(f"s_mul_i32 {s('d_tile')}, {s('d_tile')}, {s('tmp3')}")
    E(f"s_sub_u32 {s('tmp3')}, {s('tmp2')}, {s('tmp1')}")
    E(f"s_cselect_b32 {s('tmp3')}, 0, {s('tmp3')}", "max(xcd - r, 0)   (scc still: xcd < r)")
    E(f"s_mul_i32 {s('tmp3')}, {s('tmp3')}, {s('tmp0')}")
    E(f"s_add_u32 {s('d_tile')}, {s('d_tile')}, {s('tmp3')}")
    E(f"s_lshr_b32 {s('tmp3')}, {s('wg')}, 3")
    E(f"s_add_u32 {s('d_tile')}, {s('d_tile')}, {s('tmp3')}")
    E(f"s_cmp_ge_u32 {s('d_tile')}, {s('ntiles')}")
    E(f"s_cbranch_scc1 .Lend_{name}")
    W1B = 6 * 1024
    E(f"v_lshlrev_b32 v{T[3]}, 4, v{T[0]}", "16 lane")
    E(f"s_add_u32 {s('sa')}, {s('w')}, {W1B}")
    E(f"s_addc_u32 {s('sa', 1)}, {s('w', 1)}, 0")
    for i in range(3 * KS2):
        if i and i % 4 == 0:
            E(f"s_add_u32 {s('sa')}, {s('sa')}, 4096")
            E(f"s_addc_u32 {s('sa', 1)}, {s('sa', 1)}, 0")
        E(f"global_load_dwordx4 {vr('W2', 4 * i, 4)}, v{T[3]}, {s2('sa')} offset:{1024 * (i % 4)}")
    nw1 = uid("nw1")
    E(f"s_cmp_gt_u32 {s('wave')}, 5")
    E(f"s_cbranch_scc1 {nw1}")
    E(f"s_lshl_b32 {s('tmp0')}, {s('wave')}, 10")
    E(f"v_add_u32 v{T[4]}, {s('tmp0')}, v{T[3]}")
    E(f"global_load_dwordx4 v[{T[8]}:{T[8] + 3}], v{T[4]}, {s2('w')}")
    E("s_waitcnt vmcnt(0)")
    E(f"v_add_u32 v{T[4]}, {W1_OFF}, v{T[4]}")
    E(f"ds_write_b128 v{T[4]}, v[{T[8]}:{T[8] + 3}]")
    label(nw1)
    nb = uid("nb")
    E(f"s_cmp_lg_u32 {s('wave')}, 6")
    E(f"s_cbranch_scc1 {nb}")
    E(f"v_cmp_gt_u32 vcc, 24, v{T[0]}", "96 floats = 24 lanes x 16 B")
    E("s_and_saveexec_b64 s[98:99], vcc")
    E(f"global_load_dwordx4 v[{T[8]}:{T[8] + 3}], v{T[3]}, {s2('bias')}")
    E("s_waitcnt vmcnt(0)")
    E(f"v_add_u32 v{T[4]}, {BIAS_OFF}, v{T[3]}")
    E(f"ds_write_b128 v{T[4]}, v[{T[8]}:{T[8] + 3}]")
    E("s_mov_b64 exec, s[98:99]")
    label(nb)
    E(f"s_mov_b32 {s('c_ok')}, 0")
    E(f"s_mov_b32 {s('b_ok')}, 0")
    emit_decode("d")
    E(f"s_mov_b32 {s('dma_lds')}, {X0}")
    emit_dma()
    for nm in ("ok", "b", "y0", "x0"):
        E(f"s_mov_b32 {s('b_' + nm)}, {s('d_' + nm)}")
    E(f"s_add_u32 {s('d_tile')}, {s('d_tile')}, {s('G')}")
    emit_decode("d")
    E(f"s_mov_b32 {s('dma_lds')}, {X0 + BUF}")
    E("s_waitcnt vmcnt(0)")
    E("s_waitcnt lgkmcnt(0)")
    E("s_barrier")
    stamp(PH_PROLOGUE)
    loop = uid("loop")
    label(loop)
    g1 = uid("g1")
    join = uid("join")
    E(f"s_cmp_eq_u32 {s('group')}, 1")
    E(f"s_cbranch_scc1 {g1}")
    emit_phase_c(True)
    stamp(PH_C_EPI)
    emit_phase_b_dispatch()
    stamp(PH_B)
    full, w0 = uid("full"), uid("w0")
    E(f"s_and_b32 {s('tmp0')}, {s('rowok0')}, {s('rowok1')}")
    E(f"s_and_b32 {s('tmp0')}, {s('tmp0')}, {s('c_ok')}")
    E(f"s_cmp_eq_u32 {s('tmp0')}, 1")
    E(f"s_cbranch_scc1 {full}")
    E("s_waitcnt vmcnt(0)")
    E(f"s_branch {join}")
    label(full)
    E(f"s_waitcnt vmcnt({3 if W16 else 6})")
    E(f"s_branch {join}")
    label(g1)
    emit_dma()
    emit_phase_b_dispatch()
    stamp(PH_B)
    emit_phase_c(False)
    stamp(PH_C_EPI)
    nowait = uid("nw")
    E(f"s_cmp_eq_u32 {s('c_ok')}, 1")
    E(f"s_cbranch_scc1 {nowait}")
    E("s_waitcnt vmcnt(0)")
    label(nowait)
    label(join)
    E("s_waitcnt lgkmcnt(0)")
    E("s_barrier")
    stamp(PH_BARRIER)
    for nm in ("ok", "b", "y0", "x0"):
        E(f"s_mov_b32 {s('c_' + nm)}, {s('b_' + nm)}")
        E(f"s_mov_b32 {s('b_' + nm)}, {s('d_' + nm)}")
    E(f"s_add_u32 {s('d_tile')}, {s('d_tile')}, {s('G')}")
    E(f"s_mov_b32 {s('d_ok')}, 0")
    more = uid("more")
    E(f"s_cmp_eq_u32 {s('b_ok')}, 0", "no tile in stage B: none follows either")
    E(f"s_cbranch_scc1 {more}")
    emit_decode("d")
    label(more)
    E(f"s_xor_b32 {s('dma_lds')}, {s('dma_lds')}, {BUF}")
    for nm in ("cA", "cP1", "cP2", "xb", "tw"):
        E(f"v_xor_b32 {v(nm)}, {BUF}, {v(nm)}")
    E(f"s_or_b32 {s('tmp0')}, {s('c_ok')}, {s('b_ok')}")
    E(f"s_cmp_lg_u32 {s('tmp0')}, 0")
    E(f"s_cbranch_scc1 {loop}")
    label(f".Lend_{name}")
    if stamped:
        T3 = V.names["P"][0]
        E(f"s_lshl_b32 {s('tmp0')}, {s('wg')}, 3")
        E(f"s_add_u32 {s('tmp0')}, {s('tmp0')}, {s('wave')}")
        E(f"s_lshl_b32 {s('tmp0')}, {s('tmp0')}, 6")
        E(f"v_mov_b32 v{T3 + 2}, {s('tmp0')}")
        E("s_mov_b64 exec, 1")
        for k in range(6):
            E(f"v_mov_b32 v{T3}, {s('st_acc', 2 * k)}")
            E(f"v_mov_b32 v{T3 + 1}, {s('st_acc', 2 * k + 1)}")
            E(f"global_store_dwordx2 v{T3 + 2}, v[{T3}:{T3 + 1}], {s2('debug')} offset:{8 * k}")
        E("s_waitcnt vmcnt(0)")
    E("s_endpgm")
    return list(out)


def descriptor(name):
    total = (V.next + 7) // 8 * 8
    assert total <= 256 and LDS_BYTES <= 160 * 1024
    return f"""
	.rodata
	.p2align 6
	.amdhsa_kernel {name}
		.amdhsa_group_segment_fixed_size {LDS_BYTES}
		.amdhsa_private_segment_fixed_size 0
		.amdhsa_kernarg_size {ARG_BYTES}
		.amdhsa_user_sgpr_count 2
		.amdhsa_user_sgpr_kernarg_segment_ptr 1
		.amdhsa_system_sgpr_workgroup_id_x 1
		.amdhsa_system_vgpr_workitem_id 0
		.amdhsa_next_free_vgpr {total}
		.amdhsa_next_free_sgpr 100
		.amdhsa_accum_offset {total}
		.amdhsa_reserve_vcc 1
		.amdhsa_float_denorm_mode_32 3
		.amdhsa_float_denorm_mode_16_64 3
		.amdhsa_dx10_clamp 1
		.amdhsa_ieee_mode 1
	.end_amdhsa_kernel
	.text
"""


def metadata_entry(name):
    total = (V.next + 7) // 8 * 8
    return f"""  - .agpr_count:     0
    .args:
      - .offset:         0
        .size:           {ARG_BYTES}
        .value_kind:     by_value
    .group_segment_fixed_size: {LDS_BYTES}
    .kernarg_segment_align: 8
    .kernarg_segment_size: {ARG_BYTES}
    .max_flat_workgroup_size: 512
    .name:           {name}
    .private_segment_fixed_size: 0
    .sgpr_count:     106
    .symbol:         {name}.kd
    .vgpr_count:     {total}
    .wavefront_size: 64
"""


def main():
    path = sys.argv[1] if len(sys.argv) > 1 else "bottleneck_asm.s"
    text = ['\t.amdgcn_target "amdgcn-amd-amdhsa--gfx950"', "\t.text"]
    entries = []
    import os
    variants = [("bottleneck_asm_c48", False, {}), ("bottleneck_asm_c48_stamped", True, {})]
    if os.environ.get("AQ_GEN_EXPERIMENTAL") == "1":
        variants += [("bottleneck_asm_c48_nostagger", False, dict(stagger=False)), ("bottleneck_asm_c48_nostagger_stamped", True, dict(stagger=False)),
                     ("bottleneck_asm_c48_prio", False, dict(prio=3)), ("bottleneck_asm_c48_prio_stamped", True, dict(prio=3)),
                     ("bottleneck_asm_c48_nopk", False, dict(nopk=True)), ("bottleneck_asm_c48_nosilu", False, dict(nosilu=True)),
                     ("bottleneck_asm_c48_nomfma", False, dict(nomfma=True)), ("bottleneck_asm_c48_skel", False, dict(nomfma=True, nosilu=True)),
                     ("bottleneck_asm_c48_skel_nodma", False, dict(nomfma=True, nosilu=True, nodma=True)),
                     ("bottleneck_asm_c48_skel_nold", False, dict(nomfma=True, nosilu=True, nold=True)),
                     ("bottleneck_asm_c48_skel_nost", False, dict(nomfma=True, nosilu=True, nost=True)),
                     ("bottleneck_asm_c48_skel_nomem", False, dict(nomfma=True, nosilu=True, nodma=True, nold=True, nost=True)),
                     ("bottleneck_asm_c48_nomem", False, dict(nodma=True, nold=True, nost=True)),
                     ("bottleneck_asm_c48_ntst", False, dict(ntst=True)), ("bottleneck_asm_c48_ntld", False, dict(ntld=True)),
                     ("bottleneck_asm_c48_nt", False, dict(ntst=True, ntld=True))]
    for name, stamped, opt in variants:
        text += [f"\t.globl\t{name}", "\t.p2align\t8", f"\t.type\t{name},@function"]
        text += gen_kernel(name, stamped, **opt)
        entries.append(metadata_entry(name))
        text += [f".Lfend_{name}:", f"\t.size\t{name}, .Lfend_{name}-{name}", descriptor(name)]
    text.append(f"""	.amdgpu_metadata
---
amdhsa.kernels:
{"".join(entries)}amdhsa.target:   amdgcn-amd-amdhsa--gfx950
amdhsa.version:
  - 1
  - 2
...
	.end_amdgpu_metadata
""")
    with open(path, "w") as f:
        f.write("\n".join(text) + "\n")
    print(f"bottleneck_asm_c48: {V.next} VGPRs, {S.next} SGPRs, {LDS_BYTES} B LDS; wrote {path}: {sum(1 for l in text if 'v_mfma' in l)} MFMA instructions")


if __name__ == "__main__":
    main()
```

### aquaculture_amd/engine.py

```python
from __future__ import annotations

import ctypes as C
import os
from typing import Dict, List, Optional, Sequence, Tuple

import numpy as np
import torch

from . import spec as _spec
from .checkpoint import Checkpoint, pack_plan_weights

AQ_BF16, AQ_FP32, AQ_BF16_W8, AQ_F16X3 = 0, 1, 2, 3
PRECISIONS = {"bf16": AQ_BF16, "fp32": AQ_FP32, "fp8w": AQ_BF16, "f16x3": AQ_F16X3}
"""Compute precision of the single-op helpers.  fp8w = fp8 (OCP e4m3fn) weights with per-output-channel power-of-two scales, bf16
activations (quant.py): values bf16 holds exactly, so every bf16 kernel runs them as they are."""
ENGINE_PRECISIONS = {"bf16": AQ_BF16, "fp32": AQ_FP32, "fp8w": AQ_BF16_W8, "f16x3": AQ_F16X3, "fp8": AQ_BF16}
"""aq_model_desc.precision.  AQ_BF16_W8 computes as AQ_BF16; kernels with an fp8-weight stream (the planar 3x3) load the e4m3 codes."""
_DTYPE_CODE = {"act": 0, "f32": 1, "u8": 2}

LIB_PATH = os.path.join(os.path.dirname(os.path.abspath(__file__)), "csrc", "libaqengine.so")


class aq_tensor_desc(C.Structure):
    _fields_ = [("channels", C.c_int32), ("down", C.c_int32), ("dtype", C.c_int32)]


class aq_slice(C.Structure):
    _fields_ = [("tensor", C.c_int32), ("ch_off", C.c_int32), ("channels", C.c_int32)]


class aq_op_desc(C.Structure):
    _fields_ = [("kind", C.c_int32), ("src", aq_slice), ("dst", aq_slice), ("res", aq_slice),
                ("k", C.c_int32), ("stride", C.c_int32), ("pad", C.c_int32), ("act", C.c_int32),
                ("level", C.c_int32), ("weight", C.POINTER(C.c_float)), ("bias", C.POINTER(C.c_float)),
                ("flops_per_tile", C.c_double)]


class aq_model_desc(C.Structure):
    _fields_ = [("precision", C.c_int32), ("nc", C.c_int32), ("na", C.c_int32), ("nl", C.c_int32),
                ("anchors_px", C.c_float * 2 * 8 * 3), ("stride", C.c_float * 3),
                ("head_tensor", C.c_int32 * 3), ("input_tensor", C.c_int32),
                ("n_tensors", C.c_int32), ("n_ops", C.c_int32),
                ("tensors", C.POINTER(aq_tensor_desc)), ("ops", C.POINTER(aq_op_desc))]


class aq_det(C.Structure):
    _fields_ = [("x1", C.c_float), ("y1", C.c_float), ("x2", C.c_float), ("y2", C.c_float),
                ("conf", C.c_float), ("cls", C.c_float)]


EXPORTS = (
    "aq_last_error", "aq_version", "aq_engine_create", "aq_engine_destroy", "aq_engine_workspace_bytes",
    "aq_engine_infer", "aq_engine_run_ops", "aq_engine_candidates", "aq_engine_forward_raw", "aq_engine_tensor_ptr", "aq_engine_profile",
    "aq_engine_op_times", "aq_engine_num_ops", "aq_engine_set_conv_config", "aq_engine_autotune", "aq_engine_set_tuned_table",
    "aq_engine_get_conv_config", "aq_conv_num_configs", "aq_debug_conv_stamp", "aq_debug_mfma_peak",
    "aq_conv_config_tiles", "aq_pack_conv_weights", "aq_pack_conv_weights_x3", "aq_conv2d", "aq_pack_stem_weights", "aq_stem_conv", "aq_pack_bottleneck_weights", "aq_bottleneck", "aq_pack_downblock_weights", "aq_downblock", "aq_stemdown_supported", "aq_stemdown", "aq_conv1x1_direct_supported", "aq_pack_conv1x1_direct", "aq_conv1x1_direct", "aq_conv1x1_asm_supported", "aq_pack_conv1x1_asm", "aq_conv1x1_asm", "aq_nms_opts", "aq_engine_set_nms_options",
    "aq_conv3x3s2_direct_supported", "aq_pack_conv3x3s2_direct", "aq_conv3x3s2_direct",
    "aq_conv3x3_pl_supported", "aq_conv3x3_pl_asm_family", "aq_pack_conv3x3_pl", "aq_conv3x3_pl", "aq_conv3x3_pl_s2_supported", "aq_pack_conv3x3_pl_s2", "aq_conv3x3_pl_s2", "aq_jpeg_scratch_bytes", "aq_jpeg_idct_rgb", "aq_f32_to_e4m3", "aq_conv1x1_direct_f8out", "aq_absmax_bf16", "aq_engine_calibrate_amax", "aq_engine_set_fp8_scales", "aq_engine_last_launch", "aq_conv3x3_pl_f8_supported", "aq_pack_conv3x3_pl_f8", "aq_conv3x3_pl_f8", "aq_conv3x3_pl_w8_supported", "aq_pack_conv3x3_pl_w8", "aq_conv3x3_pl_w8", "aq_head_decode_supported", "aq_pack_head_weights", "aq_head_decode", "aq_head_counts_gather", "aq_preprocess_s2d", "aq_sppf_pool",
    "aq_upsample2x", "aq_letterbox_u8", "aq_letterbox_tiles_u8", "aq_format_label_rows", "aq_detect_decode", "aq_nms_scratch_bytes", "aq_nms", "aq_jpeg_huffman_decode", "aq_write_label_files",
    "aq_augment_geometry", "aq_augment_taps", "aq_stem_conv_scaled", "aq_preprocess_s2d_scaled", "aq_head_decode_aug", "aq_detect_decode_aug",
    "aq_engine_workspace_bytes_augment", "aq_engine_infer_augment", "aq_engine_forward_raw_augment", "aq_engine_last_launch_augment",
)

_lib = None


def load_library(path: str = LIB_PATH) -> C.CDLL:
    global _lib
    if _lib is not None:
        return _lib
    if path == LIB_PATH and os.environ.get("AQ_ENGINE_LIB"):
        path = os.environ["AQ_ENGINE_LIB"]
    if not os.path.exists(path):
        raise RuntimeError(f"{path} not found: build it with `python -m aquaculture_amd.build` "
                           "(there is no CPU/PyTorch fallback for the detect path)")
    lib = C.CDLL(path)
    vp, i32, f32, sz = C.c_void_p, C.c_int, C.c_float, C.c_size_t
    lib.aq_last_error.restype = C.c_char_p
    lib.aq_engine_create.argtypes = [C.POINTER(aq_model_desc), i32, C.POINTER(vp)]
    lib.aq_engine_destroy.argtypes = [vp]
    lib.aq_engine_destroy.restype = None
    lib.aq_engine_workspace_bytes.argtypes = [vp, i32, i32, i32, C.POINTER(sz)]
    lib.aq_engine_infer.argtypes = [vp, vp, i32, i32, i32, vp, sz, vp, vp, f32, f32, i32, vp]
    lib.aq_engine_run_ops.argtypes = [vp, vp, i32, i32, i32, vp, sz, i32, i32, f32, f32, i32, vp, vp, vp]
    lib.aq_engine_candidates.argtypes = [vp, C.POINTER(vp), C.POINTER(vp), C.POINTER(vp), C.POINTER(i32)]
    lib.aq_engine_forward_raw.argtypes = [vp, vp, i32, i32, i32, vp, sz, vp, vp]
    lib.aq_engine_tensor_ptr.argtypes = [vp, i32, C.POINTER(vp), C.POINTER(i32), C.POINTER(i32), C.POINTER(i32), C.POINTER(i32)]
    lib.aq_engine_profile.argtypes = [vp, i32, i32]
    lib.aq_engine_op_times.argtypes = [vp, C.POINTER(f32), i32, C.POINTER(i32)]
    lib.aq_engine_num_ops.argtypes = [vp]
    lib.aq_engine_set_conv_config.argtypes = [vp, i32, i32]
    lib.aq_engine_autotune.argtypes = [vp, vp, i32, i32, i32, vp, sz, i32, vp]
    lib.aq_engine_get_conv_config.argtypes = [vp, i32]
    lib.aq_engine_last_launch.argtypes = [vp, i32, C.POINTER(i32), C.POINTER(i32)]
    lib.aq_jpeg_huffman_decode.argtypes = [vp, vp, i32, vp, vp, vp, vp]
    lib.aq_write_label_files.argtypes = [C.c_char_p, C.POINTER(C.c_char_p), C.POINTER(f32), C.POINTER(C.c_longlong), i32, i32, i32]
    lib.aq_write_label_files.restype = C.c_long
    lib.aq_engine_set_tuned_table.argtypes = [vp, i32, i32, i32, C.POINTER(i32), i32]
    lib.aq_engine_calibrate_amax.argtypes = [vp, vp, i32, i32, i32, vp, sz, C.POINTER(f32), i32, vp]
    lib.aq_engine_set_fp8_scales.argtypes = [vp, C.POINTER(f32), i32]
    lib.aq_conv1x1_direct_f8out.argtypes = [vp, i32, i32, vp, i32, i32, i32, i32, vp, vp, C.c_longlong, i32, f32, vp]
    lib.aq_absmax_bf16.argtypes = [vp, i32, i32, i32, C.c_longlong, vp, vp]
    lib.aq_debug_conv_stamp.argtypes = [vp, sz]
    lib.aq_debug_mfma_peak.argtypes = [i32, i32, vp, vp]
    lib.aq_conv_config_tiles.argtypes = [i32, C.POINTER(i32), C.POINTER(i32)]
    lib.aq_pack_conv_weights.argtypes = [C.POINTER(f32), i32, i32, i32, i32, vp, C.POINTER(sz), vp]
    lib.aq_pack_conv_weights_x3.argtypes = [C.POINTER(f32), C.POINTER(f32), i32, i32, i32, vp, C.POINTER(sz), vp, C.POINTER(sz), vp]
    lib.aq_conv2d.argtypes = [vp, i32, i32, i32, vp, i32, i32, i32, vp, i32, i32, vp, vp,
                              i32, i32, i32, i32, i32, i32, i32, i32, i32, vp, vp]
    lib.aq_pack_stem_weights.argtypes = [C.POINTER(f32), i32, i32, vp, C.POINTER(sz), vp]
    lib.aq_stem_conv.argtypes = [vp, vp, i32, i32, i32, vp, vp, i32, i32, i32, i32, i32, vp]
    lib.aq_pack_bottleneck_weights.argtypes = [C.POINTER(f32), C.POINTER(f32), i32, vp, C.POINTER(sz), vp]
    lib.aq_bottleneck.argtypes = [vp, i32, i32, vp, i32, i32, i32, vp, vp, i32, i32, i32, i32, vp]
    lib.aq_pack_downblock_weights.argtypes = [C.POINTER(f32), C.POINTER(f32), vp, C.POINTER(sz), vp]
    lib.aq_downblock.argtypes = [vp, i32, i32, vp, i32, i32, vp, vp, i32, i32, i32, vp]
    lib.aq_conv1x1_direct_supported.argtypes = [i32, i32]
    lib.aq_pack_conv1x1_direct.argtypes = [C.POINTER(f32), i32, i32, vp, C.POINTER(sz), vp]
    lib.aq_conv1x1_direct.argtypes = [vp, i32, i32, vp, i32, i32, i32, i32, vp, vp, C.c_longlong, i32, vp]
    lib.aq_nms_opts.argtypes = [vp, i32, i32, i32, i32, f32, f32, i32, vp, vp, i32, vp, vp, vp, i32, C.c_ulonglong, C.c_ulonglong, vp]
    lib.aq_engine_set_nms_options.argtypes = [vp, i32, C.c_ulonglong, C.c_ulonglong]
    lib.aq_conv1x1_asm_supported.argtypes = [i32, i32]
    lib.aq_pack_conv1x1_asm.argtypes = [C.POINTER(f32), i32, i32, vp, C.POINTER(sz), vp]
    lib.aq_conv1x1_asm.argtypes = [vp, i32, i32, vp, i32, i32, i32, i32, vp, vp, C.c_longlong, i32, vp]
    lib.aq_conv3x3s2_direct_supported.argtypes = [i32, i32]
    lib.aq_pack_conv3x3s2_direct.argtypes = [C.POINTER(f32), i32, i32, vp, C.POINTER(sz), vp]
    lib.aq_conv3x3s2_direct.argtypes = [vp, i32, i32, vp, i32, i32, i32, i32, vp, vp, i32, i32, i32, i32, vp]
    lib.aq_conv3x3_pl_supported.argtypes = [i32, i32]
    lib.aq_conv3x3_pl_asm_family.argtypes = [i32]
    lib.aq_pack_conv3x3_pl.argtypes = [C.POINTER(f32), i32, i32, vp, C.POINTER(sz), vp]
    lib.aq_conv3x3_pl.argtypes = [vp, C.c_longlong, C.c_longlong, i32, vp, i32, i32, i32, vp, i32, i32, vp, vp, i32, i32, i32, i32, vp]
    lib.aq_conv3x3_pl_w8.argtypes = lib.aq_conv3x3_pl.argtypes
    lib.aq_pack_conv3x3_pl_w8.argtypes = [C.POINTER(C.c_float), C.POINTER(C.c_float), i32, i32, vp, C.POINTER(C.c_size_t), vp, vp]
    lib.aq_conv3x3_pl_w8_supported.argtypes = [i32] * 5
    lib.aq_jpeg_scratch_bytes.argtypes = [i32, i32, i32]
    lib.aq_jpeg_scratch_bytes.restype = sz
    lib.aq_jpeg_idct_rgb.argtypes = [vp, vp, vp, i32, i32, i32, vp, vp, vp]
    lib.aq_f32_to_e4m3.argtypes = [f32]
    lib.aq_f32_to_e4m3.restype = C.c_ubyte
    lib.aq_conv3x3_pl_f8_supported.argtypes = [i32] * 5
    lib.aq_pack_conv3x3_pl_f8.argtypes = [C.POINTER(f32), C.POINTER(f32), i32, i32, f32, vp, C.POINTER(sz), vp, vp]
    lib.aq_conv3x3_pl_f8.argtypes = [vp, i32, i32, i32, vp, i32, i32, i32, vp, i32, i32, vp, vp, i32, i32, i32, i32, vp]
    lib.aq_conv3x3_pl_s2_supported.argtypes = [i32] * 5
    lib.aq_pack_conv3x3_pl_s2.argtypes = [C.POINTER(f32), i32, i32, vp, C.POINTER(sz), vp]
    lib.aq_conv3x3_pl_s2.argtypes = [vp, i32, i32, i32, vp, i32, i32, i32, vp, vp, i32, i32, i32, i32, vp]
    lib.aq_preprocess_s2d.argtypes = [vp, vp, i32, i32, i32, i32, vp]
    lib.aq_sppf_pool.argtypes = [vp, i32, i32, i32, i32, i32, i32, i32, vp]
    lib.aq_upsample2x.argtypes = [vp, i32, i32, vp, i32, i32, i32, i32, i32, i32, i32, vp]
    lib.aq_letterbox_u8.argtypes = [vp, i32, i32, i32, vp, i32, i32, i32, i32, i32, i32, vp, vp, vp]
    lib.aq_letterbox_tiles_u8.argtypes = [vp, C.c_longlong, C.c_longlong, vp, vp, i32, i32, i32, vp, i32, i32, i32, i32, i32, i32, vp, vp, vp]
    lib.aq_format_label_rows.argtypes = [C.POINTER(f32), i32, i32, C.c_char_p, sz]
    lib.aq_format_label_rows.restype = C.c_long
    lib.aq_detect_decode.argtypes = [C.POINTER(vp), i32, i32, i32, i32, i32, i32, C.POINTER(f32), C.POINTER(f32),
                                     vp, f32, vp, vp, vp, i32, vp]
    lib.aq_nms_scratch_bytes.argtypes = [i32, i32]
    lib.aq_nms_scratch_bytes.restype = sz
    lib.aq_nms.argtypes = [vp, i32, i32, i32, i32, f32, f32, i32, vp, vp, i32, vp, vp, vp, vp]
    lib.aq_augment_geometry.argtypes = [i32, i32, i32, vp, C.POINTER(i32)]
    lib.aq_augment_taps.argtypes = [i32, i32, i32, vp]
    lib.aq_stem_conv_scaled.argtypes = [vp, i32, i32, vp, vp, i32, i32, vp, i32, i32, i32, vp, vp, i32, i32, i32, i32, i32, vp]
    lib.aq_preprocess_s2d_scaled.argtypes = [vp, i32, i32, vp, vp, i32, i32, vp, i32, i32, i32, i32, vp]
    lib.aq_head_decode_aug.argtypes = [vp, i32, i32, i32, vp, i32, i32, i32, i32, f32, C.POINTER(f32), i32, i32, f32, f32, f32, vp, vp, vp, i32, i32, vp]
    lib.aq_detect_decode_aug.argtypes = [C.POINTER(vp), i32, i32, i32, i32, i32, i32, C.POINTER(f32), C.POINTER(f32), i32, i32, i32, f32, f32,
                                         vp, f32, vp, vp, vp, i32, vp]
    lib.aq_engine_workspace_bytes_augment.argtypes = [vp, i32, i32, i32, C.POINTER(sz)]
    lib.aq_engine_infer_augment.argtypes = lib.aq_engine_infer.argtypes
    lib.aq_engine_forward_raw_augment.argtypes = lib.aq_engine_forward_raw.argtypes
    lib.aq_engine_last_launch_augment.argtypes = [vp, i32, i32, C.POINTER(i32), C.POINTER(i32)]
    _lib = lib
    return lib


def _check(rc: int) -> None:
    if rc != 0:
        raise RuntimeError(f"libaqengine error {rc}: {load_library().aq_last_error().decode()}")


def _stream_ptr() -> int:
    return torch.cuda.current_stream().cuda_stream


def _require_gpu() -> None:
    if not torch.cuda.is_available():
        raise RuntimeError("aquaculture_amd needs a ROCm GPU (MI355X/gfx950); there is no CPU fallback")


def _act_dtype(precision: int) -> torch.dtype:
    return torch.float32 if precision in (AQ_FP32, AQ_F16X3) else torch.bfloat16


class Engine:

    def __init__(self, ck: Checkpoint, precision: str = "bf16", device: int = 0, fused_stem: bool = True,
                 fused_bottleneck: Optional[bool] = None, fp8_calibration=None):
        _require_gpu()
        self.lib = load_library()
        self.ck = ck
# ... 423 lines not shown
    B = int(offs.shape[0])
    xt, yt, (nw, nh, top, left, H, W) = _letterbox_tables(H0, W0, new_shape, stride, auto, scene.device)
    offs_dev = torch.from_numpy(offs).to(scene.device)
    out = torch.empty((B, H, W, 3), dtype=torch.uint8, device=scene.device)
    _check(lib.aq_letterbox_tiles_u8(scene.data_ptr(), Hs * row_b, row_b, offs_dev.data_ptr(), offs.ctypes.data, B, H0, W0, out.data_ptr(),
                                     H, W, nw, nh, top, left, xt.data_ptr(), yt.data_ptr(), _stream_ptr()))
    return out


def format_label_rows(rows: np.ndarray, save_conf: bool = True) -> bytes:
    lib = load_library()
    rows = np.ascontiguousarray(rows, dtype=np.float32)
    n = rows.shape[0]
    if n == 0:
        return b""
    buf = C.create_string_buffer(n * 6 * 16)
    k = lib.aq_format_label_rows(rows.ctypes.data_as(C.POINTER(C.c_float)), n, int(save_conf), buf, len(buf))
    if k < 0:
        buf = C.create_string_buffer(-k + 1)
        k = lib.aq_format_label_rows(rows.ctypes.data_as(C.POINTER(C.c_float)), n, int(save_conf), buf, len(buf))
    return buf.raw[:k]


def write_label_files(labels_dir: str, stems, rows: np.ndarray, offsets: np.ndarray, save_conf: bool = True, fsync: bool = False) -> int:
    lib = load_library()
    rows = np.ascontiguousarray(rows, dtype=np.float32)
    offsets = np.ascontiguousarray(offsets, dtype=np.int64)
    n = len(stems)
    assert offsets.shape[0] == n + 1 and (rows.shape[0] == 0 or rows.shape[1] == 6)
    arr = (C.c_char_p * n)(*[os.fsencode(s_) for s_ in stems])
    k = lib.aq_write_label_files(os.fsencode(labels_dir), arr, rows.ctypes.data_as(C.POINTER(C.c_float)), offsets.ctypes.data_as(C.POINTER(C.c_longlong)), n,
                                 int(save_conf), int(fsync))
    if k < 0:
        raise OSError(f"could not write the label file of {stems[-1 - k]} in {labels_dir}")
    return int(k)


def stem_conv_nhwc(tiles_u8: torch.Tensor, w_oihw: torch.Tensor, bias: torch.Tensor, act: bool = True, precision: str = "bf16") -> torch.Tensor:
    _require_gpu()
    lib = load_library()
    prec = PRECISIONS[precision]
    B, H, W, _ = tiles_u8.shape
    cout = w_oihw.shape[0]
    w = np.ascontiguousarray(w_oihw.permute(0, 2, 3, 1).float().cpu().numpy())
    n = C.c_size_t()
    wp = w.ctypes.data_as(C.POINTER(C.c_float))
    _check(lib.aq_pack_stem_weights(wp, cout, prec, None, C.byref(n), None))
    wbuf = torch.empty(n.value, dtype=torch.uint8, device=tiles_u8.device)
    _check(lib.aq_pack_stem_weights(wp, cout, prec, wbuf.data_ptr(), C.byref(n), _stream_ptr()))
    bbuf = torch.zeros(64, dtype=torch.float32, device=tiles_u8.device)
    bbuf[:cout] = bias.float().to(tiles_u8.device)
    out = torch.empty((B, H // 2, W // 2, cout), dtype=_act_dtype(prec), device=tiles_u8.device)
    _check(lib.aq_stem_conv(tiles_u8.data_ptr(), out.data_ptr(), cout, 0, cout, wbuf.data_ptr(), bbuf.data_ptr(), B, H, W, int(act), prec,
                            _stream_ptr()))
    torch.cuda.current_stream().synchronize()
    return out


def bottleneck_nhwc(x: torch.Tensor, w1_oihw: torch.Tensor, b1: torch.Tensor, w2_oihw: torch.Tensor, b2: torch.Tensor,
                    shortcut: bool = True, out: Optional[torch.Tensor] = None) -> torch.Tensor:
    _require_gpu()
    lib = load_library()
    assert x.dtype == torch.bfloat16 and x.stride(3) == 1
    B, H, W, c = x.shape
    ld = x.stride(2)
    assert x.stride(1) == W * ld and x.stride(0) == H * W * ld, "x must be a channel slice of a dense NHWC tensor"
    w1 = np.ascontiguousarray(w1_oihw.permute(0, 2, 3, 1).float().cpu().numpy())
    w2 = np.ascontiguousarray(w2_oihw.permute(0, 2, 3, 1).float().cpu().numpy())
    n = C.c_size_t()
    p1, p2 = w1.ctypes.data_as(C.POINTER(C.c_float)), w2.ctypes.data_as(C.POINTER(C.c_float))
    _check(lib.aq_pack_bottleneck_weights(p1, p2, c, None, C.byref(n), None))
    wbuf = torch.empty(n.value, dtype=torch.uint8, device=x.device)
    _check(lib.aq_pack_bottleneck_weights(p1, p2, c, wbuf.data_ptr(), C.byref(n), _stream_ptr()))
    bbuf = torch.cat([b1.float(), b2.float()]).to(x.device).contiguous()
    if out is None:
        out = torch.empty((B, H, W, c), dtype=torch.bfloat16, device=x.device)
    old = out.stride(2)
    _check(lib.aq_bottleneck(x.data_ptr(), ld, 0, out.data_ptr(), old, 0, c, wbuf.data_ptr(), bbuf.data_ptr(), B, H, W, int(shortcut),
                             _stream_ptr()))
    torch.cuda.current_stream().synchronize()
    return out


def downblock_nhwc(x: torch.Tensor, wa_oihw: torch.Tensor, ba: torch.Tensor, wb_oihw: torch.Tensor, bb: torch.Tensor,
                   out: Optional[torch.Tensor] = None) -> torch.Tensor:
    _require_gpu()
    lib = load_library()
    assert x.dtype == torch.bfloat16 and x.stride(3) == 1 and x.shape[3] == 48
    B, H, W, _ = x.shape
    ld = x.stride(2)
    assert x.stride(1) == W * ld and x.stride(0) == H * W * ld, "x must be a channel slice of a dense NHWC tensor"
    wa = np.ascontiguousarray(wa_oihw.permute(0, 2, 3, 1).float().cpu().numpy())
    wb = np.ascontiguousarray(wb_oihw.permute(0, 2, 3, 1).float().cpu().numpy())
    n = C.c_size_t()
    pa, pb = wa.ctypes.data_as(C.POINTER(C.c_float)), wb.ctypes.data_as(C.POINTER(C.c_float))
    _check(lib.aq_pack_downblock_weights(pa, pb, None, C.byref(n), None))
    wbuf = torch.empty(n.value, dtype=torch.uint8, device=x.device)
    _check(lib.aq_pack_downblock_weights(pa, pb, wbuf.data_ptr(), C.byref(n), _stream_ptr()))
    bbuf = torch.cat([ba.float(), bb.float()]).to(x.device).contiguous()
    if out is None:
        out = torch.empty((B, H // 2, W // 2, 96), dtype=torch.bfloat16, device=x.device)
    _check(lib.aq_downblock(x.data_ptr(), ld, 0, out.data_ptr(), out.stride(2), 0, wbuf.data_ptr(), bbuf.data_ptr(), B, H, W, _stream_ptr()))
    torch.cuda.current_stream().synchronize()
    return out


CONV_CFG_DIRECT1X1 = 1000
CONV_CFG_ASM1X1 = 1004
CONV_CFG_DIRECT3X3S2 = 1001
CONV_CFG_PL3X3 = 1002
CONV_CFG_PL3X3S2 = 1003
CONV_CFG_ONE_TILE_PER_WG = 4096


def conv3x3_pl_nhwc(x: torch.Tensor, w_oihw: torch.Tensor, bias: torch.Tensor, act: bool = True,
                    residual: Optional[torch.Tensor] = None, out: Optional[torch.Tensor] = None, w8: bool = False) -> torch.Tensor:
    _require_gpu()
    lib = load_library()
    assert x.dtype == torch.bfloat16 and x.stride(3) == 1
    B, H, W, cin = x.shape
    cout = w_oihw.shape[0]
    ld = x.stride(2)
    assert x.stride(1) == W * ld and x.stride(0) == H * W * ld, "x must be a channel slice of a dense NHWC tensor"
    w = np.ascontiguousarray(w_oihw.permute(0, 2, 3, 1).float().cpu().numpy())
    n = C.c_size_t()
    wp = w.ctypes.data_as(C.POINTER(C.c_float))
    if w8:
        if not lib.aq_conv3x3_pl_w8_supported(cin, cout, B, H, W):
            raise RuntimeError("aq_conv3x3_pl_w8 does not support this shape")
        bh = np.ascontiguousarray(bias.float().cpu().numpy())
        bp = bh.ctypes.data_as(C.POINTER(C.c_float))
        _check(lib.aq_pack_conv3x3_pl_w8(wp, bp, cin, cout, None, C.byref(n), None, None))
        wbuf = torch.empty(n.value, dtype=torch.uint8, device=x.device)
        bbuf = torch.empty(2048, dtype=torch.float32, device=x.device)
        _check(lib.aq_pack_conv3x3_pl_w8(wp, bp, cin, cout, wbuf.data_ptr(), C.byref(n), bbuf.data_ptr(), _stream_ptr()))
    else:
        _check(lib.aq_pack_conv3x3_pl(wp, cin, cout, None, C.byref(n), None))
        wbuf = torch.empty(n.value, dtype=torch.uint8, device=x.device)
        _check(lib.aq_pack_conv3x3_pl(wp, cin, cout, wbuf.data_ptr(), C.byref(n), _stream_ptr()))
        bbuf = bias.float().to(x.device).contiguous()
    if out is None:
        out = torch.empty((B, H, W, cout), dtype=torch.bfloat16, device=x.device)
    assert out.stride(3) == 1 and (residual is None or residual.stride(3) == 1)
    _check((lib.aq_conv3x3_pl_w8 if w8 else lib.aq_conv3x3_pl)(x.data_ptr(), ld * 2, 16, cin, out.data_ptr(), out.stride(2), 0, cout,
                             residual.data_ptr() if residual is not None else None, residual.stride(2) if residual is not None else 0, 0,
                             wbuf.data_ptr(), bbuf.data_ptr(), B, H, W, int(act), _stream_ptr()))
    torch.cuda.current_stream().synchronize()
    return out


def conv1x1_direct_nhwc(x: torch.Tensor, w_oihw: torch.Tensor, bias: torch.Tensor, act: bool = True, out: Optional[torch.Tensor] = None) -> torch.Tensor:
    _require_gpu()
    lib = load_library()
    assert x.dtype == torch.bfloat16 and x.stride(-1) == 1
    cin, cout = x.shape[-1], w_oihw.shape[0]
    ld = x.stride(-2)
    npix = x.numel() // cin
    w = np.ascontiguousarray(w_oihw.reshape(cout, cin).float().cpu().numpy())
    n = C.c_size_t()
    wp = w.ctypes.data_as(C.POINTER(C.c_float))
    _check(lib.aq_pack_conv1x1_direct(wp, cin, cout, None, C.byref(n), None))
    wbuf = torch.empty(n.value, dtype=torch.uint8, device=x.device)
    _check(lib.aq_pack_conv1x1_direct(wp, cin, cout, wbuf.data_ptr(), C.byref(n), _stream_ptr()))
    bbuf = bias.float().to(x.device).contiguous()
    if out is None:
        out = torch.empty(x.shape[:-1] + (cout,), dtype=torch.bfloat16, device=x.device)
# ... 281 lines not shown
```

### include/aq_engine.h

```cpp
#ifndef AQ_ENGINE_H
#define AQ_ENGINE_H

#include <stddef.h>
#include <stdint.h>

#ifdef __cplusplus
extern "C" {
#endif

typedef enum aq_status {
    AQ_OK = 0,
    AQ_ERR_INVALID = -1,
    AQ_ERR_HIP = -2,
    AQ_ERR_NOMEM = -3,
    AQ_ERR_WORKSPACE = -4
} aq_status;

typedef enum aq_precision {
    AQ_BF16 = 0,
    AQ_FP32 = 1,
    AQ_BF16_W8 = 2,
    AQ_F16X3 = 3
} aq_precision;

// ... 26 lines not shown
typedef struct aq_model_desc {
    int32_t precision;
    int32_t nc, na, nl;
    float anchors_px[3][8][2];
    float stride[3];
    int32_t head_tensor[3];
    int32_t input_tensor;
    int32_t n_tensors, n_ops;
    const aq_tensor_desc* tensors;
    const aq_op_desc* ops;
} aq_model_desc;

typedef struct aq_det { float x1, y1, x2, y2, conf, cls; } aq_det;

typedef struct aq_engine aq_engine;

const char* aq_last_error(void);
int aq_version(void);

int aq_engine_create(const aq_model_desc* desc, int device_ordinal, aq_engine** out);
void aq_engine_destroy(aq_engine* e);
int aq_engine_workspace_bytes(aq_engine* e, int max_batch, int H, int W, size_t* bytes);
int aq_engine_infer(aq_engine* e, const uint8_t* tiles_dev, int B, int H, int W,
                    void* workspace_dev, size_t workspace_bytes,
                    aq_det* dets_dev, int32_t* counts_dev,
                    float conf_thres, float iou_thres, int max_det, void* stream);
int aq_engine_forward_raw(aq_engine* e, const uint8_t* tiles_dev, int B, int H, int W,
                          void* workspace_dev, size_t workspace_bytes, float* pred_dev, void* stream);
int aq_engine_run_ops(aq_engine* e, const uint8_t* tiles_dev, int B, int H, int W, void* workspace_dev, size_t workspace_bytes,
                      int first, int last, float conf_thres, float iou_thres, int max_det, aq_det* dets_dev, int32_t* counts_dev,
                      void* stream);
int aq_engine_tensor_ptr(aq_engine* e, int tensor, void** ptr, int* channels, int* h, int* w, int* elem_bytes);
int aq_engine_profile(aq_engine* e, int enable, int ring);
int aq_engine_candidates(aq_engine* e, void** cand_dev, void** rows_dev, void** counts_dev, int* cap);
int aq_engine_op_times(aq_engine* e, float* ms_out, int n_ops, int* calls_recorded);
int aq_engine_num_ops(aq_engine* e);
int aq_engine_set_conv_config(aq_engine* e, int op, int cfg);
int aq_engine_autotune(aq_engine* e, const uint8_t* tiles_dev, int B, int H, int W,
                       void* workspace_dev, size_t workspace_bytes, int reps, void* stream);
int aq_engine_calibrate_amax(aq_engine* e, const uint8_t* tiles_dev, int B, int H, int W, void* workspace_dev, size_t workspace_bytes,
                             float* amax_host, int n_ops, void* stream);
int aq_engine_set_fp8_scales(aq_engine* e, const float* act_scale, int n_ops);
int aq_engine_get_conv_config(aq_engine* e, int op);
enum {
    AQ_FAM_NONE = 0,
    AQ_FAM_IGEMM_OR_HALO = 1,
    AQ_FAM_PL3X3 = 2,
    AQ_FAM_PL3X3_W8 = 3,
    AQ_FAM_PL3X3S2 = 4,
    AQ_FAM_PL3X3_F8 = 5,
    AQ_FAM_DIRECT1X1 = 6,
    AQ_FAM_DIRECT1X1_F8OUT = 7,
    AQ_FAM_DIRECT3X3S2 = 8,
    AQ_FAM_BOTTLENECK = 9,
    AQ_FAM_DOWNBLOCK = 10,
    AQ_FAM_STEM = 11,
    AQ_FAM_HEAD_DECODE = 12,
    AQ_FAM_ASM1X1 = 13
};
int aq_engine_last_launch(aq_engine* e, int op, int* family, int* cfg);
int aq_engine_set_tuned_table(aq_engine* e, int B, int H, int W, const int* cfgs, int n_ops);
int aq_conv_num_configs(void);
int aq_debug_conv_stamp(void* buf_dev, size_t bytes);
int aq_debug_mfma_peak(int blocks, int iters, void* out_dev, void* stream);
int aq_conv_config_tiles(int cfg, int* bm, int* bn);

int aq_pack_conv_weights(const float* w_krsc_host, int cout, int k, int cin, int precision,
                         void* packed_dev, size_t* bytes, void* stream);
int aq_pack_conv_weights_x3(const float* w_krsc_host, const float* bias_host, int cout, int k, int cin, void* packed_dev, size_t* bytes,
                            float* bias_scale_dev, size_t* bias_floats, void* stream);
int aq_conv2d(const void* in_dev, int in_ld, int in_choff, int cin,
              void* out_dev, int out_ld, int out_choff, int cout,
              const void* res_dev, int res_ld, int res_choff,
              const void* packed_w_dev, const float* bias_dev,
              int B, int H, int W, int k, int stride, int pad, int act,
              int precision, int out_f32, const void* zero_page_dev, void* stream);
int aq_pack_stem_weights(const float* w_krsc_host, int cout, int precision, void* packed_dev, size_t* bytes, void* stream);
int aq_stem_conv(const uint8_t* tiles_dev, void* out_dev, int out_ld, int out_choff, int cout, const void* packed_w_dev,
                 const float* bias_dev, int B, int H, int W, int act, int precision, void* stream);

int aq_pack_bottleneck_weights(const float* w1_host, const float* w2_host, int C, void* packed_dev, size_t* bytes, void* stream);
int aq_bottleneck(const void* in_dev, int in_ld, int in_choff, void* out_dev, int out_ld, int out_choff, int C,
                  const void* packed_w_dev, const float* bias_dev, int B, int H, int W, int shortcut, void* stream);

int aq_pack_downblock_weights(const float* wa_host, const float* wb_host, void* packed_dev, size_t* bytes, void* stream);
int aq_downblock(const void* in_dev, int in_ld, int in_choff, void* out_dev, int out_ld, int out_choff,
                 const void* packed_w_dev, const float* bias_dev, int B, int H, int W, void* stream);
int aq_stemdown_supported(int Hi, int Wi);
int aq_stemdown(const uint8_t* tiles_dev, void* out_dev, int out_ld, int out_choff, const void* stem_w_dev, const float* stem_bias_dev,
                const void* packed_w_dev, const float* bias_dev, int B, int Hi, int Wi, void* stream);

#define AQ_CONV_CFG_DIRECT1X1 1000
#define AQ_CONV_CFG_ONE_TILE_PER_WG 4096
int aq_conv1x1_direct_supported(int cin, int cout);
int aq_pack_conv1x1_direct(const float* w_host, int cin, int cout, void* packed_dev, size_t* bytes, void* stream);
int aq_conv1x1_direct(const void* in_dev, int in_ld, int in_choff, void* out_dev, int out_ld, int out_choff, int cin, int cout,
                      const void* packed_w_dev, const float* bias_dev, long long npix, int act, void* stream);

#define AQ_CONV_CFG_ASM1X1 1004
int aq_conv1x1_asm_supported(int cin, int cout);
int aq_pack_conv1x1_asm(const float* w_host, int cin, int cout, void* packed_dev, size_t* bytes, void* stream);
int aq_conv1x1_asm(const void* in_dev, int in_ld, int in_choff, void* out_dev, int out_ld, int out_choff, int cin, int cout,
                   const void* packed_w_dev, const float* bias_dev, long long npix, int act, void* stream);

#define AQ_CONV_CFG_DIRECT3X3S2 1001
int aq_conv3x3s2_direct_supported(int cin, int cout);
int aq_pack_conv3x3s2_direct(const float* w_host, int cin, int cout, void* packed_dev, size_t* bytes, void* stream);
int aq_conv3x3s2_direct(const void* in_dev, int in_ld, int in_choff, void* out_dev, int out_ld, int out_choff, int cin, int cout,
                        const void* packed_w_dev, const float* bias_dev, int B, int H, int W, int act, void* stream);
#define AQ_CONV_CFG_PL3X3 1002
int aq_conv3x3_pl_supported(int cin, int cout);
int aq_conv3x3_pl_asm_family(int nb);
int aq_pack_conv3x3_pl(const float* w_krsc_host, int cin, int cout, void* packed_dev, size_t* bytes, void* stream);
int aq_conv3x3_pl(const void* in_dev, long long in_pixel_stride_b, long long in_group_stride_b, int cin,
                  void* out_dev, int out_ld, int out_choff, int cout, const void* res_dev, int res_ld, int res_choff,
                  const void* packed_w_dev, const float* bias_dev, int B, int H, int W, int act, void* stream);
#define AQ_CONV_CFG_PL3X3S2 1003
int aq_conv3x3_pl_s2_supported(int cin, int cout, int B, int H, int W);
int aq_pack_conv3x3_pl_s2(const float* w_krsc_host, int cin, int cout, void* packed_dev, size_t* bytes, void* stream);
int aq_conv3x3_pl_s2(const void* in_dev, int in_ld, int in_choff, int cin, void* out_dev, int out_ld, int out_choff, int cout,
                     const void* packed_w_dev, const float* bias_dev, int B, int H, int W, int act, void* stream);
int aq_conv1x1_direct_f8out(const void* in_dev, int in_ld, int in_choff, void* out_dev, int out_pitch_bytes, int out_byte_off, int cin, int cout,
                            const void* packed_w_dev, const float* bias_dev, long long npix, int act, float out_scale, void* stream);
int aq_absmax_bf16(const void* t_dev, int ld, int choff, int c, long long npix, float* out_dev, void* stream);
unsigned char aq_f32_to_e4m3(float v);
int aq_conv3x3_pl_f8_supported(int cin, int cout, int B, int H, int W);
int aq_pack_conv3x3_pl_f8(const float* w_krsc_host, const float* bias_host, int cin, int cout, float act_scale, void* packed_dev,
                          size_t* bytes, float* scale_bias_dev, void* stream);
int aq_conv3x3_pl_f8(const void* in_dev, int in_ld, int in_choff, int cin, void* out_dev, int out_ld, int out_choff, int cout,
                     const void* res_dev, int res_ld, int res_choff, const void* packed_w_dev, const float* scale_bias_dev,
                     int B, int H, int W, int act, void* stream);
int aq_conv3x3_pl_w8_supported(int cin, int cout, int B, int H, int W);
int aq_pack_conv3x3_pl_w8(const float* w_krsc_host, const float* bias_host, int cin, int cout, void* packed_dev, size_t* bytes,
                          float* scale_bias_dev, void* stream);
int aq_conv3x3_pl_w8(const void* in_dev, long long in_sp, long long in_ss, int cin, void* out_dev, int out_ld, int out_choff,
                     int cout, const void* res_dev, int res_ld, int res_choff, const void* packed_w8_dev,
                     const float* scale_bias_dev, int B, int H, int W, int act, void* stream);
int aq_preprocess_s2d(const uint8_t* tiles_dev, void* out_dev, int B, int H, int W, int precision, void* stream);
int aq_letterbox_u8(const uint8_t* src_dev, int B, int H0, int W0, uint8_t* dst_dev, int H, int W, int new_w, int new_h,
                    int top, int left, const int32_t* xtab_dev, const int32_t* ytab_dev, void* stream);
int aq_letterbox_tiles_u8(const uint8_t* scene_dev, long long scene_bytes, long long row_bytes, const long long* tile_off_dev,
                          const long long* tile_off_host, int B, int H0, int W0, uint8_t* dst_dev, int H, int W, int new_w, int new_h,
                          int top, int left, const int32_t* xtab_dev, const int32_t* ytab_dev, void* stream);
size_t aq_jpeg_scratch_bytes(int B, int H, int W);
int aq_jpeg_idct_rgb(const int16_t* coef_dev, const long long* coef_off_dev, const uint16_t* qt_dev, int B, int H, int W,
                     void* scratch_dev, uint8_t* out_dev, void* stream);
int aq_jpeg_huffman_decode(const void* streams_dev, const void* segs_dev, int nseg, const void* tabsets_dev, void* coef_dev,
                           void* status_dev, void* stream);
int aq_sppf_pool(void* buf_dev, int ld, int ch_off, int c, int B, int H, int W, int precision, void* stream);
int aq_upsample2x(const void* in_dev, int in_ld, int in_choff, void* out_dev, int out_ld, int out_choff,
                  int c, int B, int H, int W, int precision, void* stream);
int aq_head_decode_supported(int cin, int na, int nc);
int aq_pack_head_weights(const float* w_host, const float* bias_host, int cin, int cout, void* packed_dev, size_t* bytes, void* stream);
int aq_head_decode(const void* in_dev, int in_ld, int in_choff, int cin, const void* packed_dev, int B, int ny, int nx,
                   int cand_off, float stride, const float* anchors_px, int nc, int na, float conf_thres,
                   int32_t* cand_dev, float* cand_rows_dev, int32_t* cand_count_dev, int count_stride, int cand_cap, void* stream);
int aq_head_counts_gather(const int32_t* wide_dev, int count_stride, int32_t* compact_dev, int B, void* stream);

int aq_detect_decode(const float* const head_dev[3], int head_ld, int B, int H, int W, int nc, int na,
                     const float* anchors_px , const float* stride ,
                     float* pred_dev, float conf_thres, int32_t* cand_dev, float* cand_rows_dev,
                     int32_t* cand_count_dev, int cand_cap, void* stream);
size_t aq_nms_scratch_bytes(int B, int N);
int aq_nms(const float* rows_dev, int rows_per_tile, int B, int N, int nc, float conf_thres, float iou_thres,
           int max_det, const int32_t* cand_dev, const int32_t* cand_count_dev, int cand_cap,
           void* scratch_dev, aq_det* dets_dev, int32_t* counts_dev, void* stream);
// ... 47 lines not shown
```

Measured before the change: 16490.

## Fuse C3 bottleneck with following cv3 1x1 conv into one asm kernel

Adds a tail variant of the C48 bottleneck assembly kernel. It takes the bottleneck's 48-channel result and the concat partner (cv2 output) loaded from global memory, then runs the 96→96 1x1 cv3 conv with bias and SiLU inside the same kernel. The engine detects eligible bottleneck+conv pairs at creation, packs the combined weights, and skips the separate conv launch. This removes the concat tensor's write and re-read and one launch per C3 block. In exchange the kernel needs more LDS and registers, and the pattern matching and env gating add complexity.

```diff
diff --git a/aquaculture_amd/csrc/bottleneck.hip b/aquaculture_amd/csrc/bottleneck.hip
--- a/aquaculture_amd/csrc/bottleneck.hip
+++ b/aquaculture_amd/csrc/bottleneck.hip
@@ -609,6 +609,86 @@
     }
 }
 
+struct BtlTailArgs {
+    BtlAsmArgs a;
+    const char* cat;
+    int cat_ld_b, pad2;
+};
+static_assert(sizeof(BtlTailArgs) == 112, "kernel argument block");
+constexpr size_t kBtlTailWBytes = kBtlAsmWBytes + (size_t)18 * 1024;
+
+void btl_tail_pack_w3(const float* w3, bf16_t* dst) {
+    for (int m = 0; m < 6; ++m)
+        for (int s = 0; s < 3; ++s)
+            for (int lane = 0; lane < 64; ++lane, dst += 8) {
+                const int co = 16 * m + (lane & 15), c0 = 32 * s + 8 * (lane >> 4);
+                for (int e = 0; e < 8; ++e) dst[e] = aq_f2bf(w3[(size_t)co * 96 + c0 + e]);
+            }
+}
+
+}
+
+extern "C" int aq_bottleneck_c3tail_supported(int B, int H, int W, int in_ld, int cat_ld, int out_ld) {
+    if (!btl_asm_fits(48, B, H, W, in_ld, out_ld)) return 0;
+    return (long long)B * H * W * cat_ld * 2 < (1LL << 31) && in_ld % 8 == 0 && cat_ld % 8 == 0 && out_ld % 8 == 0;
+}
+
+extern "C" int aq_pack_bottleneck_c3tail_weights(const float* w1_host, const float* w2_host, const float* w3_host, void* packed_dev, size_t* bytes,
+                                                  void* stream) {
+    AQ_REQUIRE(w1_host && w2_host && w3_host && bytes, "pack_bottleneck_c3tail: null pointer");
+    *bytes = kBtlTailWBytes;
+    if (!packed_dev) return AQ_OK;
+    bf16_t* host = (bf16_t*)calloc(1, *bytes);
+    AQ_REQUIRE(host, "pack_bottleneck_c3tail: out of host memory");
+    btl_asm_pack(w1_host, w2_host, host);
+    btl_tail_pack_w3(w3_host, (bf16_t*)((char*)host + kBtlAsmWBytes));
+    hipError_t e = hipMemcpyAsync(packed_dev, host, *bytes, hipMemcpyHostToDevice, (hipStream_t)stream);
+    if (e == hipSuccess) e = hipStreamSynchronize((hipStream_t)stream);
+    free(host);
+    AQ_CHECK_HIP(e);
+    return AQ_OK;
+}
+
+extern "C" int aq_bottleneck_c3tail(const void* in_dev, int in_ld, int in_choff, const void* cat_dev, int cat_ld, int cat_choff, void* out_dev,
+                                    int out_ld, int out_choff, const void* packed_w_dev, const float* bias_dev, int B, int H, int W, int shortcut,
+                                    void* stream) {
+    AQ_REQUIRE(in_dev && cat_dev && out_dev && packed_w_dev && bias_dev, "bottleneck_c3tail: null pointer");
+    AQ_REQUIRE(B > 0 && H > 0 && W > 0, "bottleneck_c3tail: empty input");
+    AQ_REQUIRE(in_choff % 8 == 0 && cat_choff % 8 == 0 && out_choff % 8 == 0 && in_choff + 48 <= in_ld && cat_choff + 48 <= cat_ld &&
+                   out_choff + 96 <= out_ld, "bottleneck_c3tail: channel slices must be 8-aligned and inside their rows");
+    if (!aq_bottleneck_c3tail_supported(B, H, W, in_ld, cat_ld, out_ld)) {
+        aq_set_error("bottleneck_c3tail: unsupported geometry %d x %d x %d (or AQ_BTL_ASM=0)", B, H, W);
+        return AQ_ERR_INVALID;
+    }
+    {
+        const size_t np = (size_t)B * H * W;
+        const char* i0 = (const char*)in_dev + (size_t)in_choff * 2; const char* i1 = i0 + (np - 1) * in_ld * 2 + 96;
+        const char* c0 = (const char*)cat_dev + (size_t)cat_choff * 2; const char* c1 = c0 + (np - 1) * cat_ld * 2 + 96;
+        const char* o0 = (const char*)out_dev + (size_t)out_choff * 2; const char* o1 = o0 + (np - 1) * out_ld * 2 + 192;
+        AQ_REQUIRE((o1 <= i0 || i1 <= o0) && (o1 <= c0 || c1 <= o0), "bottleneck_c3tail: output overlaps an input");
+    }
+    int cus = 0;
+    AQ_CHECK_HIP(aq_cus(&cus));
+    BtlTailArgs t{};
+    BtlAsmArgs& a = t.a;
+    a.in = (const char*)in_dev + (size_t)in_choff * 2; a.out = (char*)out_dev + (size_t)out_choff * 2;
+    a.w = (const char*)packed_w_dev; a.bias = bias_dev;
+    a.in_ld_b = in_ld * 2; a.out_ld_b = out_ld * 2; a.B = B; a.H = H; a.W = W;
+    a.tiles_x = (W + 15) / 16;
+    a.tpi = a.tiles_x * ((H + 15) / 16);
+    a.ntiles = a.tpi * B;
+    a.shortcut = shortcut;
+    long long grid = cus;
+    if (grid > a.ntiles) grid = a.ntiles;
+    a.G = (int)grid;
+    a.magic_tpi = (unsigned)((1ULL << 32) / (unsigned)a.tpi + 1);
+    a.magic_tx = (unsigned)((1ULL << 32) / (unsigned)a.tiles_x + 1);
+    a.in_bytes = (unsigned)(((long long)B * H * W - 1) * a.in_ld_b + 96);
+    t.cat = (const char*)cat_dev + (size_t)cat_choff * 2; t.cat_ld_b = cat_ld * 2;
+    hipFunction_t fn = nullptr;
+    AQ_CHECK_HIP(aq_asm_fn(kBtlAsmCode, "bottleneck_asm_c48_tail", &fn, false));
+    AQ_CHECK_HIP(aq_asm_launch(fn, (unsigned)grid, 512, &t, sizeof t, (hipStream_t)stream));
+    return AQ_OK;
 }
 
 extern "C" int aq_pack_bottleneck_weights(const float* w1_host, const float* w2_host, int C, void* packed_dev, size_t* bytes, void* stream) {
diff --git a/aquaculture_amd/csrc/engine.cpp b/aquaculture_amd/csrc/engine.cpp
--- a/aquaculture_amd/csrc/engine.cpp
+++ b/aquaculture_amd/csrc/engine.cpp
@@ -69,6 +69,8 @@
     float act_scale = 0.0f;
     int f8_consumer = -1;
     std::vector<float> w_host, b_host;
+    void* w_tail = nullptr;
+    float* b_tail = nullptr;
 };
 
 void pack_host(const float* w, int cout, int k, int cin, int precision, std::vector<unsigned char>& out,
@@ -390,6 +392,21 @@
     return n_heads == 3;
 }
 
+bool c3tail_active(aq_engine* e, int oi, int last, int B) {
+    if (!e->packed[oi].w_tail || oi + 1 >= last || e->calib_amax || e->tuning) return false;
+    const int ci = oi + 1;
+    const PackedW& pc = e->packed[ci];
+    if (pc.direct_cfg != AQ_CONV_CFG_DIRECT1X1 || (pc.f8_consumer >= 0 && f8_pair_active(e, pc.f8_consumer, B))) return false;
+    const aq_engine::Tuned* tt = tuned_for(e);
+    const int cfg = e->conv_cfg[ci] >= 0 ? e->conv_cfg[ci] : tt ? tt->cfg[ci] : -1;
+    if (cfg != AQ_CONV_CFG_DIRECT1X1) return false;
+    const aq_op_desc& b = e->ops[oi];
+    const aq_op_desc& c = e->ops[ci];
+    const TensorPlace& pl = e->place[b.src.tensor];
+    return aq_bottleneck_c3tail_supported(B, pl.h, pl.w, e->tensors[b.src.tensor].channels, e->tensors[c.src.tensor].channels,
+                                          e->tensors[c.dst.tensor].channels) != 0;
+}
+
 struct AugRun {
     int pass;
     const aq_augment_pass* ps;
@@ -438,6 +455,7 @@
             heads_started = true;
             ++heads_done;
         }
+    int tail_conv = -1;
     for (int oi = first; oi < last; ++oi) {
         const aq_op_desc& op = e->ops[oi];
         if (ev) AQ_CHECK_HIP(hipEventRecord(ev[oi], stream));
@@ -457,6 +475,10 @@
                 rc = aq_preprocess_s2d(tiles, tptr(e, ws, tiles, op.dst.tensor), B, H, W, prec, stream);
             break;
         case AQ_OP_CONV:
+            if (oi == tail_conv) {
+                note_launch(e, oi, AQ_FAM_DIRECT1X1, AQ_CONV_CFG_DIRECT1X1);
+                break;
+            }
             if (ar && op.level >= 0 && !((ar->ps->level_mask >> op.level) & 1)) {
                 note_launch(e, oi, AQ_FAM_NONE);
                 break;
@@ -510,6 +532,15 @@
         case AQ_OP_BOTTLENECK: {
             note_launch(e, oi, AQ_FAM_BOTTLENECK);
             const TensorPlace& pl = e->place[op.src.tensor];
+            if (c3tail_active(e, oi, last, B)) {
+                const aq_op_desc& c = e->ops[oi + 1];
+                rc = aq_bottleneck_c3tail(tptr(e, ws, tiles, op.src.tensor), e->tensors[op.src.tensor].channels, op.src.ch_off,
+                                          tptr(e, ws, tiles, c.src.tensor), e->tensors[c.src.tensor].channels, op.dst.channels,
+                                          tptr(e, ws, tiles, c.dst.tensor), e->tensors[c.dst.tensor].channels, c.dst.ch_off,
+                                          e->packed[oi].w_tail, e->packed[oi].b_tail, B, pl.h, pl.w, op.res.tensor >= 0, stream);
+                tail_conv = oi + 1;
+                break;
+            }
             rc = aq_bottleneck(tptr(e, ws, tiles, op.src.tensor), e->tensors[op.src.tensor].channels, op.src.ch_off,
                                tptr(e, ws, tiles, op.dst.tensor), e->tensors[op.dst.tensor].channels, op.dst.ch_off,
                                op.src.channels, e->packed[oi].w, e->packed[oi].bias, B, pl.h, pl.w, op.res.tensor >= 0, stream);
@@ -736,6 +767,36 @@
         aq_set_error("engine_create: zero page allocation failed");
         return fail(AQ_ERR_NOMEM);
     }
+    const char* use_tail = getenv("AQ_C3TAIL");
+    for (size_t oi = 0; d->precision == AQ_BF16 && !(use_tail && *use_tail == '0') && oi + 1 < e->ops.size(); ++oi) {
+        const aq_op_desc& b = e->ops[oi];
+        const aq_op_desc& c = e->ops[oi + 1];
+        if (b.kind != AQ_OP_BOTTLENECK || c.kind != AQ_OP_CONV || !b.weight || !b.bias || !c.weight || !c.bias) continue;
+        if (b.src.channels != 48 || b.dst.channels != 48 || b.k != 3 || b.dst.tensor < 0 || b.dst.tensor >= d->n_tensors || b.dst.ch_off != 0 ||
+            e->tensors[b.dst.tensor].channels != 96 || b.src.tensor == b.dst.tensor)
+            continue;
+        if (c.k != 1 || c.stride != 1 || c.act != 1 || c.res.tensor >= 0 || c.level >= 0 || c.src.tensor != b.dst.tensor || c.src.ch_off != 0 ||
+            c.src.channels != 96 || c.dst.channels != 96 || c.dst.tensor < 0 || c.dst.tensor >= d->n_tensors || c.dst.tensor == c.src.tensor ||
+            c.dst.tensor == b.src.tensor || c.dst.ch_off % 8 || e->tensors[c.dst.tensor].channels % 8 || e->tensors[c.dst.tensor].dtype != AQ_T_ACT)
+            continue;
+        bool read_later = false;
+        for (size_t oj = oi + 2; oj < e->ops.size(); ++oj)
+            for (const aq_slice* s : {&e->ops[oj].src, &e->ops[oj].res})
+                if (s->tensor == b.dst.tensor && s->ch_off < b.dst.ch_off + b.dst.channels && b.dst.ch_off < s->ch_off + s->channels) read_later = true;
+        if (read_later) continue;
+        PackedW& pw = e->packed[oi];
+        size_t nb = 0;
+        float bias[192];
+        memcpy(bias, b.bias, sizeof(float) * 96);
+        memcpy(bias + 96, c.bias, sizeof(float) * 96);
+        if (aq_pack_bottleneck_c3tail_weights(b.weight, b.weight + (size_t)48 * 48, c.weight, nullptr, &nb, nullptr) != AQ_OK ||
+            hipMalloc(&pw.w_tail, nb) != hipSuccess || hipMalloc((void**)&pw.b_tail, sizeof bias) != hipSuccess ||
+            aq_pack_bottleneck_c3tail_weights(b.weight, b.weight + (size_t)48 * 48, c.weight, pw.w_tail, &nb, nullptr) != AQ_OK ||
+            hipMemcpy(pw.b_tail, bias, sizeof bias, hipMemcpyHostToDevice) != hipSuccess) {
+            aq_set_error("engine_create: C3 tail weight upload failed (op %zu)", oi);
+            return fail(AQ_ERR_HIP);
+        }
+    }
     for (size_t oi = 0; oi < e->ops.size(); ++oi) {
         aq_op_desc& op = e->ops[oi];
         for (const aq_slice* s : {&op.src, &op.dst}) {
@@ -936,6 +997,8 @@
         if (pw.w_f8) (void)hipFree(pw.w_f8);
         if (pw.sb_f8) (void)hipFree(pw.sb_f8);
         if (pw.sb_pl8) (void)hipFree(pw.sb_pl8);
+        if (pw.w_tail) (void)hipFree(pw.w_tail);
+        if (pw.b_tail) (void)hipFree(pw.b_tail);
         if (pw.bias) (void)hipFree(pw.bias);
     }
     if (e->zero_page) (void)hipFree(e->zero_page);
diff --git a/aquaculture_amd/csrc/gen_bottleneck_asm.py b/aquaculture_amd/csrc/gen_bottleneck_asm.py
--- a/aquaculture_amd/csrc/gen_bottleneck_asm.py
+++ b/aquaculture_amd/csrc/gen_bottleneck_asm.py
@@ -20,6 +20,12 @@
 ARG = dict(inp=0, out=8, w=16, bias=24, in_ld=32, out_ld=36, B=40, H=44, W=48, tiles_x=52, tpi=56, ntiles=60, shortcut=64, G=68,
            magic_tpi=72, magic_tx=76, in_bytes=80, pad=84, debug=88)
 ARG_BYTES = 96
+
+BIAS3_OFF = BIAS_OFF + 384
+W3_OFF = BIAS_OFF + 768
+LDS_BYTES_TAIL = W3_OFF + 18 * 1024
+ARG_TAIL = dict(cat=96, cat_ld=104)
+ARG_BYTES_TAIL = 112
 
 
 class Regs:
@@ -79,14 +85,18 @@
 V.alloc("P", 28, 4)
 
 
+S_TAIL = dict(cat=(S.names["st_acc"][0], 2), cat_ld=(S.names["st_acc"][0] + 2, 1), crow0=(S.names["st_acc"][0] + 4, 2),
+              crow1=(S.names["st_acc"][0] + 6, 2))
+
+
 def s(name, i=0):
-    b, n = S.names[name]
+    b, n = S.names[name] if name in S.names else S_TAIL[name]
     assert i < n
     return f"s{b + i}"
 
 
 def s2(name, i=0):
-    b, n = S.names[name]
+    b, n = S.names[name] if name in S.names else S_TAIL[name]
     assert i + 1 < n and (b + i) % 2 == 0
     return f"s[{b + i}:{b + i + 1}]"
 
@@ -120,7 +130,7 @@
 out = []
 _uid = [0]
 STAMPED = [False]
-OPT = dict(stagger=True, nosilu=False, nomfma=False, nopk=False, nodma=False, nold=False, nost=False, prio=0, ntst=False, ntld=False)
+OPT = dict(stagger=True, nosilu=False, nomfma=False, nopk=False, nodma=False, nold=False, nost=False, prio=0, ntst=False, ntld=False, tail=False)
 PH_PROLOGUE, PH_DMA, PH_B, PH_C_MFMA, PH_C_EPI, PH_BARRIER = range(6)
 
 
@@ -328,6 +338,86 @@
     label(skip)
 
 
+def tail_r(i):
+    return V.names["ACC"][0] + i
+
+
+def emit_tail_cat_loads():
+    R = tail_r
+    tid = V.names["tid"][0]
+    E(f"v_lshrrev_b32 v{R(65)}, 1, v{tid}")
+    E(f"v_and_b32 v{R(65)}, 0x18, v{R(65)}", "8 g")
+    E(f"v_mad_u32_u24 v{R(64)}, {v('l15')}, {s('cat_ld')}, v{R(65)}", "l15 cat_ld + 8 g: c 4 g")
+    E(f"v_add_u32 v{R(65)}, v{R(64)}, v{R(65)}", "+ 8 g more: c 16 + 8 g (at offset 32)")
+    for j in range(2):
+        E(f"s_mov_b64 exec, {s2('mask' + str(j))}")
+        E(f"global_load_dwordx2 v[{R(26 + 8 * j)}:{R(27 + 8 * j)}], v{R(64)}, {s2('crow' + str(j))}")
+        E(f"global_load_dwordx4 v[{R(28 + 8 * j)}:{R(31 + 8 * j)}], v{R(65)}, {s2('crow' + str(j))} offset:32")
+    E("s_mov_b64 exec, -1")
+    return 4
+
+
+def emit_tail_gemm():
+    R = tail_r
+    E("s_waitcnt vmcnt(0)", "the cv2 values")
+    pairs = [(R(12 * j + k), R(12 * j + 2 + k)) for j in range(2) for k in range(2)] + [(R(24 + 8 * j + k), R(26 + 8 * j + k)) for j in range(2) for k in range(2)]
+    for op in ("v_permlane32_swap_b32", "v_permlane16_swap_b32"):
+        for a, b in pairs:
+            E(f"{op} v{a}, v{b}")
+
+    def bfrag(j, k):
+        base = (R(12 * j), R(24 + 8 * j), R(28 + 8 * j))[k]
+        return f"v[{base}:{base + 3}]"
+
+    def acc3(j, i):
+        return f"v[{R(40 + 4 * (2 * j + i))}:{R(43 + 4 * (2 * j + i))}]"
+
+    ring = [R(56), R(60), R(64)]
+    silu_temps = [R(4 + i) for i in range(8)] + [R(16 + i) for i in range(8)]
+    E(f"s_mov_b32 {s('sa')}, 0xffff0000", "lanes with odd g")
+    E(f"s_mov_b32 {s('sa', 1)}, 0xffff0000")
+    E("s_nop 1", "hz: VALU write -> MFMA read")
+    for t in range(3):
+        frags = [(i, k) for i in range(2) for k in range(3)]
+
+        def fread(f):
+            i, k = frags[f]
+            r = ring[f % 3]
+            E(f"ds_read_b128 v[{r}:{r + 3}], {v('w1a')} offset:{W3_OFF - W1_OFF + 1024 * (3 * (2 * t + i) + k)}")
+
+        for i in range(2):
+            E(f"ds_read_b128 v[{R(4 + 4 * i)}:{R(7 + 4 * i)}], {v('bb')} offset:{BIAS3_OFF - BIAS_OFF + 64 * (2 * t + i)}", "b3")
+        fread(0)
+        fread(1)
+        for f in range(6):
+            if f + 2 < 6:
+                fread(f + 2)
+            E(f"s_waitcnt lgkmcnt({min(5, f + 2) - f})")
+            i, k = frags[f]
+            for j in range(2):
+                E(f"v_mfma_f32_16x16x32_bf16 {acc3(j, i)}, v[{ring[f % 3]}:{ring[f % 3] + 3}], {bfrag(j, k)}, {'0' if k == 0 else acc3(j, i)}")
+        E("s_nop 15", "hz: MFMA result -> VALU read")
+        regs = [R(40 + i) for i in range(16)]
+        for q in range(0, 16, 2):
+            bq = R(4 + 4 * ((q // 4) % 2) + q % 4)
+            E(f"v_pk_add_f32 v[{regs[q]}:{regs[q] + 1}], v[{regs[q]}:{regs[q] + 1}], v[{bq}:{bq + 1}]")
+        emit_silu(regs, silu_temps)
+        for q in range(0, 16, 2):
+            E(f"v_pk_mul_f32 v[{regs[q]}:{regs[q] + 1}], v[{regs[q]}:{regs[q] + 1}], v[{silu_temps[q]}:{silu_temps[q] + 1}]")
+        for j in range(2):
+            for q in range(4):
+                E(f"v_cvt_pk_bf16_f32 v{R(16 + 4 * j + q)}, v{regs[8 * j + 2 * q]}, v{regs[8 * j + 2 * q] + 1}")
+        E(f"v_cndmask_b32 v{R(4)}, 0, 24, {s2('sa')}")
+        E(f"v_add_u32 v{R(4)}, v{R(4)}, {v('vout')}")
+        for j in range(2):
+            E(f"v_permlane16_swap_b32 v{R(16 + 4 * j)}, v{R(18 + 4 * j)}")
+            E(f"v_permlane16_swap_b32 v{R(17 + 4 * j)}, v{R(19 + 4 * j)}")
+        for j in range(2):
+            E(f"s_mov_b64 exec, {s2('mask' + str(j))}")
+            E(f"global_store_dwordx4 v{R(4)}, v[{R(16 + 4 * j)}:{R(19 + 4 * j)}], {s2('orow' + str(j))} offset:{64 * t}")
+        E("s_mov_b64 exec, -1")
+
+
 def emit_phase_c(dma_inside):
     skip = uid("pc")
     if dma_inside:
@@ -354,7 +444,7 @@
     E(f"s_add_u32 {s('tmp1')}, {s('tmp1')}, {s('tmp0')}")
     E(f"s_mul_i32 {s('tmp1')}, {s('tmp1')}, {s('W')}")
     E(f"s_add_u32 {s('tmp1')}, {s('tmp1')}, {s('c_x0')}", "pixel index of (row 0, x0)")
-    for nm, ld, base in (("orow", "out_ld", "out"), ("irow", "in_ld", "inp")):
+    for nm, ld, base in (("orow", "out_ld", "out"), ("irow", "in_ld", "inp")) + ((("crow", "cat_ld", "cat"),) if OPT["tail"] else ()):
         E(f"s_mul_i32 {s('tmp2')}, {s('tmp1')}, {s(ld)}")
         E(f"s_mul_hi_u32 {s('tmp3')}, {s('tmp1')}, {s(ld)}")
         E(f"s_add_u32 {s(nm + '0')}, {s(base)}, {s('tmp2')}")
@@ -410,17 +500,20 @@
         E("s_setprio 0")
     stamp(PH_C_MFMA)
     E("s_nop 15", "hz: MFMA result -> VALU read")
+    ncat = 0
+    if OPT["tail"]:
+        ncat = emit_tail_cat_loads()
     if dma_inside:
         w0, wd = uid("w0"), uid("wd")
         E(f"s_cmp_eq_u32 {s('d_ok')}, 0")
         E(f"s_cbranch_scc1 {w0}")
-        E("s_waitcnt vmcnt(4)", "shortcut values (the four LDS-DMA instructions behind them stay in flight)")
+        E(f"s_waitcnt vmcnt({4 + ncat})", "shortcut values (the four LDS-DMA instructions behind them stay in flight)")
         E(f"s_branch {wd}")
         label(w0)
-        E("s_waitcnt vmcnt(0)")
+        E(f"s_waitcnt vmcnt({ncat})")
         label(wd)
     else:
-        E("s_waitcnt vmcnt(0)", "shortcut values (and, vmcnt being in order, this interval's LDS-DMA and the previous tile's stores)")
+        E(f"s_waitcnt vmcnt({ncat})", "shortcut values (and, vmcnt being in order, this interval's LDS-DMA and the previous tile's stores)")
     stamp(PH_DMA)
     temps = [P0 + 12 + i for i in range(12)]
     plain, done = uid("pl"), uid("dn")
@@ -474,6 +567,11 @@
                     E(f"global_store_dwordx4 v{temps[7]}, v[{A0}:{A0 + 3}], {s2('orow0')} offset:64")
                     E("s_mov_b64 exec, -1")
                 continue
+            if OPT["tail"]:
+                for k in range(6):
+                    d = A0 + 12 * j + k if k < 4 else F0 + 8 * j + k - 4
+                    E(f"v_cvt_pk_bf16_f32 v{d}, v{regs[2 * k]}, v{regs[2 * k] + 1}")
+                continue
             for k in range(6):
                 E(f"v_cvt_pk_bf16_f32 v{temps[k]}, v{regs[2 * k]}, v{regs[2 * k] + 1}")
             E(f"s_mov_b64 exec, {s2('mask' + str(j))}")
@@ -483,6 +581,8 @@
         if with_sc:
             E(f"s_branch {done}")
     label(done)
+    if OPT["tail"]:
+        emit_tail_gemm()
     stamp(PH_C_EPI)
     label(skip)
 
@@ -494,7 +594,8 @@
     global out
     out = []
     STAMPED[0] = stamped
-    OPT.update(dict(stagger=True, nosilu=False, nomfma=False, nopk=False, nodma=False, nold=False, nost=False, prio=0, ntst=False, ntld=False))
+    assert not (stamped and opt.get("tail")), "the tail kernel keeps its scalars in the stamp accumulators"
+    OPT.update(dict(stagger=True, nosilu=False, nomfma=False, nopk=False, nodma=False, nold=False, nost=False, prio=0, ntst=False, ntld=False, tail=False))
     OPT.update(opt)
     _kernel_no[0] += 1
     _uid[0] = 100000 * _kernel_no[0]
@@ -507,6 +608,9 @@
     E(f"s_load_dwordx8 s[{b0}:{b0 + 7}], {s2('karg')}, 0x20", "in_ld .. ntiles")
     E(f"s_load_dwordx4 s[{b0 + 8}:{b0 + 11}], {s2('karg')}, 0x40", "shortcut, G, magic_tpi, magic_tx")
     E(f"s_load_dwordx4 s[{b0 + 12}:{b0 + 15}], {s2('karg')}, 0x50", "in_bytes, pad, debug")
+    if OPT["tail"]:
+        E(f"s_load_dwordx2 {s2('cat')}, {s2('karg')}, {ARG_TAIL['cat']:#x}", "cv2's half of the concat buffer")
+        E(f"s_load_dword {s('cat_ld')}, {s2('karg')}, {ARG_TAIL['cat_ld']:#x}")
     T = [V.names["P"][0] + i for i in range(28)]
     E(f"v_and_b32 v{T[0]}, 63, {v('tid')}", "lane")
     E(f"v_lshrrev_b32 v{T[1]}, 6, {v('tid')}")
@@ -617,7 +721,10 @@
     nb = uid("nb")
     E(f"s_cmp_lg_u32 {s('wave')}, 6")
     E(f"s_cbranch_scc1 {nb}")
-    E(f"v_cmp_gt_u32 vcc, 24, v{T[0]}", "96 floats = 24 lanes x 16 B")
+    if OPT["tail"]:
+        E(f"v_cmp_gt_u32 vcc, 48, v{T[0]}", "b1 | b2 | b3: 192 floats = 48 lanes x 16 B")
+    else:
+        E(f"v_cmp_gt_u32 vcc, 24, v{T[0]}", "96 floats = 24 lanes x 16 B")
     E("s_and_saveexec_b64 s[98:99], vcc")
     E(f"global_load_dwordx4 v[{T[8]}:{T[8] + 3}], v{T[3]}, {s2('bias')}")
     E("s_waitcnt vmcnt(0)")
@@ -625,6 +732,20 @@
     E(f"ds_write_b128 v{T[4]}, v[{T[8]}:{T[8] + 3}]")
     E("s_mov_b64 exec, s[98:99]")
     label(nb)
+    if OPT["tail"]:
+        for f0 in (0, 8, 16):
+            nw3 = uid("nw3")
+            if f0 == 16:
+                E(f"s_cmp_gt_u32 {s('wave')}, 1")
+                E(f"s_cbranch_scc1 {nw3}")
+            E(f"s_lshl_b32 {s('tmp0')}, {s('wave')}, 10")
+            E(f"s_add_u32 {s('tmp0')}, {s('tmp0')}, {(6 + 42 + f0) * 1024}")
+            E(f"v_add_u32 v{T[4]}, {s('tmp0')}, v{T[3]}")
+            E(f"global_load_dwordx4 v[{T[8]}:{T[8] + 3}], v{T[4]}, {s2('w')}")
+            E("s_waitcnt vmcnt(0)")
+            E(f"v_add_u32 v{T[4]}, {W3_OFF - (6 + 42) * 1024}, v{T[4]}")
+            E(f"ds_write_b128 v{T[4]}, v[{T[8]}:{T[8] + 3}]")
+            label(nw3)
     E(f"s_mov_b32 {s('c_ok')}, 0")
     E(f"s_mov_b32 {s('b_ok')}, 0")
     emit_decode("d")
@@ -707,16 +828,16 @@
     return list(out)
 
 
-def descriptor(name):
+def descriptor(name, lds=LDS_BYTES, arg_bytes=ARG_BYTES):
     total = (V.next + 7) // 8 * 8
-    assert total <= 256 and LDS_BYTES <= 160 * 1024
+    assert total <= 256 and lds <= 160 * 1024
     return f"""
 	.rodata
 	.p2align 6
 	.amdhsa_kernel {name}
-		.amdhsa_group_segment_fixed_size {LDS_BYTES}
+		.amdhsa_group_segment_fixed_size {lds}
 		.amdhsa_private_segment_fixed_size 0
-		.amdhsa_kernarg_size {ARG_BYTES}
+		.amdhsa_kernarg_size {arg_bytes}
 		.amdhsa_user_sgpr_count 2
 		.amdhsa_user_sgpr_kernarg_segment_ptr 1
 		.amdhsa_system_sgpr_workgroup_id_x 1
@@ -734,16 +855,16 @@
 """
 
 
-def metadata_entry(name):
+def metadata_entry(name, lds=LDS_BYTES, arg_bytes=ARG_BYTES):
     total = (V.next + 7) // 8 * 8
     return f"""  - .agpr_count:     0
     .args:
       - .offset:         0
-        .size:           {ARG_BYTES}
+        .size:           {arg_bytes}
         .value_kind:     by_value
-    .group_segment_fixed_size: {LDS_BYTES}
+    .group_segment_fixed_size: {lds}
     .kernarg_segment_align: 8
-    .kernarg_segment_size: {ARG_BYTES}
+    .kernarg_segment_size: {arg_bytes}
     .max_flat_workgroup_size: 512
     .name:           {name}
     .private_segment_fixed_size: 0
@@ -772,11 +893,13 @@
                      ("bottleneck_asm_c48_nomem", False, dict(nodma=True, nold=True, nost=True)),
                      ("bottleneck_asm_c48_ntst", False, dict(ntst=True)), ("bottleneck_asm_c48_ntld", False, dict(ntld=True)),
                      ("bottleneck_asm_c48_nt", False, dict(ntst=True, ntld=True))]
+    variants.append(("bottleneck_asm_c48_tail", False, dict(tail=True)))
     for name, stamped, opt in variants:
         text += [f"\t.globl\t{name}", "\t.p2align\t8", f"\t.type\t{name},@function"]
         text += gen_kernel(name, stamped, **opt)
-        entries.append(metadata_entry(name))
-        text += [f".Lfend_{name}:", f"\t.size\t{name}, .Lfend_{name}-{name}", descriptor(name)]
+        sizes = (LDS_BYTES_TAIL, ARG_BYTES_TAIL) if opt.get("tail") else (LDS_BYTES, ARG_BYTES)
+        entries.append(metadata_entry(name, *sizes))
+        text += [f".Lfend_{name}:", f"\t.size\t{name}, .Lfend_{name}-{name}", descriptor(name, *sizes)]
     text.append(f"""	.amdgpu_metadata
 ---
 amdhsa.kernels:
diff --git a/aquaculture_amd/engine.py b/aquaculture_amd/engine.py
--- a/aquaculture_amd/engine.py
+++ b/aquaculture_amd/engine.py
@@ -54,7 +54,7 @@
     "aq_engine_infer", "aq_engine_run_ops", "aq_engine_candidates", "aq_engine_forward_raw", "aq_engine_tensor_ptr", "aq_engine_profile",
     "aq_engine_op_times", "aq_engine_num_ops", "aq_engine_set_conv_config", "aq_engine_autotune", "aq_engine_set_tuned_table",
     "aq_engine_get_conv_config", "aq_conv_num_configs", "aq_debug_conv_stamp", "aq_debug_mfma_peak",
-    "aq_conv_config_tiles", "aq_pack_conv_weights", "aq_pack_conv_weights_x3", "aq_conv2d", "aq_pack_stem_weights", "aq_stem_conv", "aq_pack_bottleneck_weights", "aq_bottleneck", "aq_pack_downblock_weights", "aq_downblock", "aq_stemdown_supported", "aq_stemdown", "aq_conv1x1_direct_supported", "aq_pack_conv1x1_direct", "aq_conv1x1_direct", "aq_conv1x1_asm_supported", "aq_pack_conv1x1_asm", "aq_conv1x1_asm", "aq_nms_opts", "aq_engine_set_nms_options",
+    "aq_conv_config_tiles", "aq_pack_conv_weights", "aq_pack_conv_weights_x3", "aq_conv2d", "aq_pack_stem_weights", "aq_stem_conv", "aq_pack_bottleneck_weights", "aq_bottleneck", "aq_bottleneck_c3tail_supported", "aq_pack_bottleneck_c3tail_weights", "aq_bottleneck_c3tail", "aq_pack_downblock_weights", "aq_downblock", "aq_stemdown_supported", "aq_stemdown", "aq_conv1x1_direct_supported", "aq_pack_conv1x1_direct", "aq_conv1x1_direct", "aq_conv1x1_asm_supported", "aq_pack_conv1x1_asm", "aq_conv1x1_asm", "aq_nms_opts", "aq_engine_set_nms_options",
     "aq_conv3x3s2_direct_supported", "aq_pack_conv3x3s2_direct", "aq_conv3x3s2_direct",
     "aq_conv3x3_pl_supported", "aq_conv3x3_pl_asm_family", "aq_pack_conv3x3_pl", "aq_conv3x3_pl", "aq_conv3x3_pl_s2_supported", "aq_pack_conv3x3_pl_s2", "aq_conv3x3_pl_s2", "aq_jpeg_scratch_bytes", "aq_jpeg_idct_rgb", "aq_f32_to_e4m3", "aq_conv1x1_direct_f8out", "aq_absmax_bf16", "aq_engine_calibrate_amax", "aq_engine_set_fp8_scales", "aq_engine_last_launch", "aq_conv3x3_pl_f8_supported", "aq_pack_conv3x3_pl_f8", "aq_conv3x3_pl_f8", "aq_conv3x3_pl_w8_supported", "aq_pack_conv3x3_pl_w8", "aq_conv3x3_pl_w8", "aq_head_decode_supported", "aq_pack_head_weights", "aq_head_decode", "aq_head_counts_gather", "aq_preprocess_s2d", "aq_sppf_pool",
     "aq_upsample2x", "aq_letterbox_u8", "aq_letterbox_tiles_u8", "aq_format_label_rows", "aq_detect_decode", "aq_nms_scratch_bytes", "aq_nms", "aq_jpeg_huffman_decode", "aq_write_label_files",
@@ -112,6 +112,9 @@
     lib.aq_stem_conv.argtypes = [vp, vp, i32, i32, i32, vp, vp, i32, i32, i32, i32, i32, vp]
     lib.aq_pack_bottleneck_weights.argtypes = [C.POINTER(f32), C.POINTER(f32), i32, vp, C.POINTER(sz), vp]
     lib.aq_bottleneck.argtypes = [vp, i32, i32, vp, i32, i32, i32, vp, vp, i32, i32, i32, i32, vp]
+    lib.aq_bottleneck_c3tail_supported.argtypes = [i32, i32, i32, i32, i32, i32]
+    lib.aq_pack_bottleneck_c3tail_weights.argtypes = [C.POINTER(f32), C.POINTER(f32), C.POINTER(f32), vp, C.POINTER(sz), vp]
+    lib.aq_bottleneck_c3tail.argtypes = [vp, i32, i32, vp, i32, i32, vp, i32, i32, vp, vp, i32, i32, i32, i32, vp]
     lib.aq_pack_downblock_weights.argtypes = [C.POINTER(f32), C.POINTER(f32), vp, C.POINTER(sz), vp]
     lib.aq_downblock.argtypes = [vp, i32, i32, vp, i32, i32, vp, vp, i32, i32, i32, vp]
     lib.aq_conv1x1_direct_supported.argtypes = [i32, i32]
@@ -701,6 +704,37 @@
     return out
 
 
+def pack_bottleneck_c3tail(w1_oihw: torch.Tensor, b1: torch.Tensor, w2_oihw: torch.Tensor, b2: torch.Tensor, w3_oihw: torch.Tensor,
+                           b3: torch.Tensor, device) -> Tuple[torch.Tensor, torch.Tensor]:
+    lib = load_library()
+    ws = [np.ascontiguousarray(w.permute(0, 2, 3, 1).float().cpu().numpy()) for w in (w1_oihw, w2_oihw, w3_oihw)]
+    ps = [w.ctypes.data_as(C.POINTER(C.c_float)) for w in ws]
+    n = C.c_size_t()
+    _check(lib.aq_pack_bottleneck_c3tail_weights(*ps, None, C.byref(n), None))
+    wbuf = torch.empty(n.value, dtype=torch.uint8, device=device)
+    _check(lib.aq_pack_bottleneck_c3tail_weights(*ps, wbuf.data_ptr(), C.byref(n), _stream_ptr()))
+    return wbuf, torch.cat([b1.float(), b2.float(), b3.float()]).to(device).contiguous()
+
+
+def bottleneck_c3tail_supported(B: int, H: int, W: int, in_ld: int = 48, cat_ld: int = 96, out_ld: int = 96) -> bool:
+    return bool(load_library().aq_bottleneck_c3tail_supported(B, H, W, in_ld, cat_ld, out_ld))
+
+
+def bottleneck_c3tail_nhwc(x: torch.Tensor, c: torch.Tensor, packed: Tuple[torch.Tensor, torch.Tensor], shortcut: bool = True,
+                           out: Optional[torch.Tensor] = None, sync: bool = True) -> torch.Tensor:
+    _require_gpu()
+    lib = load_library()
+    assert x.dtype == torch.bfloat16 and c.dtype == torch.bfloat16 and x.stride(3) == 1 and c.stride(3) == 1
+    B, H, W, _ = x.shape
+    if out is None:
+        out = torch.empty((B, H, W, 96), dtype=torch.bfloat16, device=x.device)
+    _check(lib.aq_bottleneck_c3tail(x.data_ptr(), x.stride(2), 0, c.data_ptr(), c.stride(2), 0, out.data_ptr(), out.stride(2), 0,
+                                    packed[0].data_ptr(), packed[1].data_ptr(), B, H, W, int(shortcut), _stream_ptr()))
+    if sync:
+        torch.cuda.current_stream().synchronize()
+    return out
+
+
 def downblock_nhwc(x: torch.Tensor, wa_oihw: torch.Tensor, ba: torch.Tensor, wb_oihw: torch.Tensor, bb: torch.Tensor,
                    out: Optional[torch.Tensor] = None) -> torch.Tensor:
     _require_gpu()
diff --git a/include/aq_engine.h b/include/aq_engine.h
--- a/include/aq_engine.h
+++ b/include/aq_engine.h
@@ -132,6 +132,13 @@
 int aq_pack_bottleneck_weights(const float* w1_host, const float* w2_host, int C, void* packed_dev, size_t* bytes, void* stream);
 int aq_bottleneck(const void* in_dev, int in_ld, int in_choff, void* out_dev, int out_ld, int out_choff, int C,
                   const void* packed_w_dev, const float* bias_dev, int B, int H, int W, int shortcut, void* stream);
+
+int aq_bottleneck_c3tail_supported(int B, int H, int W, int in_ld, int cat_ld, int out_ld);
+int aq_pack_bottleneck_c3tail_weights(const float* w1_host, const float* w2_host, const float* w3_host, void* packed_dev, size_t* bytes,
+                                      void* stream);
+int aq_bottleneck_c3tail(const void* in_dev, int in_ld, int in_choff, const void* cat_dev, int cat_ld, int cat_choff, void* out_dev,
+                         int out_ld, int out_choff, const void* packed_w_dev, const float* bias_dev, int B, int H, int W, int shortcut,
+                         void* stream);
 
 int aq_pack_downblock_weights(const float* wa_host, const float* wb_host, void* packed_dev, size_t* bytes, void* stream);
 int aq_downblock(const void* in_dev, int in_ld, int in_choff, void* out_dev, int out_ld, int out_choff,
```

Result: faster. 16790 (median of 6 runs) (+1.8%).
